# nulltea/hyper-greco

Measured on AMD Instinct MI355X. Metric: GKR prove ms, n=32768 k=16 Goldilocks; achieved HBM GB/s vs roofline, lower is better.
Workload: dtype u64; 1 GPU; GKR prove (sk_encryption_circuit.rs:444-457) of the BFV sk-enc circuit, n=32768 k=16 Goldilocks/GoldilocksExt2, a new witness every step (4 seeded synthetic witnesses in rotation), node tables resident in HBM; witnesses=4, n=32768, k=16, field=goldilocks, parallelism=dp1: one independent proof per GPU, no data-path collective, proof_bytes=149488

## Files before the change

hyper-greco_amd/csrc/kernels.hip:

```cpp
#include <hip/hip_runtime.h>
#include <cstring>
#include <algorithm>
#include <stdexcept>
#include <string>
#include <type_traits>
#include "kernels.hpp"
#include "gl_wide.hpp"
#include "derive_math.hpp"

namespace hg {
namespace dev {

constexpr int TPB = 256;

template <int CTRL, int ROW_MASK>
__device__ __forceinline__ u64 dpp_u64(u64 v) {
    u32 lo = (u32)__builtin_amdgcn_update_dpp(0, (int)(u32)v, CTRL, ROW_MASK, 0xF, false);
    u32 hi = (u32)__builtin_amdgcn_update_dpp(0, (int)(u32)(v >> 32), CTRL, ROW_MASK, 0xF, false);
    return ((u64)hi << 32) | lo;
}
__device__ __forceinline__ u64 wave_sum_u64(u64 v) {
    v = gl_add(v, dpp_u64<0x111, 0xF>(v));
    v = gl_add(v, dpp_u64<0x112, 0xF>(v));
    v = gl_add(v, dpp_u64<0x114, 0xF>(v));
    v = gl_add(v, dpp_u64<0x118, 0xF>(v));
    v = gl_add(v, dpp_u64<0x142, 0xA>(v));
    v = gl_add(v, dpp_u64<0x143, 0xC>(v));
    u32 lo = (u32)__builtin_amdgcn_readlane((int)(u32)v, 63), hi = (u32)__builtin_amdgcn_readlane((int)(u32)(v >> 32), 63);
    return ((u64)hi << 32) | lo;
}
__device__ __forceinline__ E2 wave_sum(E2 v) { return e2(wave_sum_u64(v.c0), wave_sum_u64(v.c1)); }
__device__ __forceinline__ E2 block_sum(E2 v, E2* sm) {
    v = wave_sum(v);
    int lane = threadIdx.x & 63, wave = threadIdx.x >> 6;
    __syncthreads();
    if (lane == 0) sm[wave] = v;
    __syncthreads();
    if (threadIdx.x == 0) {
        for (int w = 1; w < TPB / 64; w++) v = e2_add(v, sm[w]);
    }
    return v;
}

static size_t st_min_threads() { return 65536; }
#ifndef HG_TEST_ST_MAX_BLOCKS
#define HG_TEST_ST_MAX_BLOCKS 512
#endif
static int st_max_blocks() { return HG_TEST_ST_MAX_BLOCKS; }

static inline int grid_for(size_t work_items) {
    size_t b = (work_items + TPB - 1) / TPB;
    if (b < 1) b = 1;
    return (int)(b > (size_t)SC_MAX_BLOCKS ? SC_MAX_BLOCKS : b);
}

template <typename T> struct Val;
template <> struct Val<u64> {
    static __device__ __forceinline__ u64 add(u64 a, u64 b) { return gl_add(a, b); }
    static __device__ __forceinline__ u64 sub(u64 a, u64 b) { return gl_sub(a, b); }
    static __device__ __forceinline__ u64 mul(u64 a, u64 b) { return gl_mul(a, b); }
    static __device__ __forceinline__ E2 scale(E2 c, u64 a) { return e2_mul_f(c, a); }
    static __device__ __forceinline__ E2 fold(u64 x, u64 d, E2 r) { return e2_add_f(e2_mul_f(r, d), x); }
    static __device__ __forceinline__ E2 lift(u64 a) { return e2(a, 0); }
    static __device__ __forceinline__ u64 zero() { return 0; }
};
template <> struct Val<E2> {
    static __device__ __forceinline__ E2 add(E2 a, E2 b) { return e2_add(a, b); }
    static __device__ __forceinline__ E2 sub(E2 a, E2 b) { return e2_sub(a, b); }
    static __device__ __forceinline__ E2 mul(E2 a, E2 b) { return e2_mul(a, b); }
    static __device__ __forceinline__ E2 scale(E2 c, E2 a) { return e2_mul(c, a); }
    static __device__ __forceinline__ E2 fold(E2 x, E2 d, E2 r) { return e2_add(x, e2_mul(r, d)); }
    static __device__ __forceinline__ E2 lift(E2 a) { return a; }
    static __device__ __forceinline__ E2 zero() { return e2_zero(); }
};

typedef unsigned long long u64x2_t __attribute__((ext_vector_type(2)));
#define HG_GLOBAL(T, p) (reinterpret_cast<__attribute__((address_space(1))) T*>((unsigned long long)(p)))
template <bool GIO = true>
__device__ __forceinline__ u64x2_t load16(const void* p) {
    if constexpr (GIO) return *HG_GLOBAL(const u64x2_t, p);
    else return *reinterpret_cast<const u64x2_t*>(p);
}
template <bool GIO = true>
__device__ __forceinline__ void store16(void* p, u64 a, u64 b) {
    u64x2_t w; w.x = a; w.y = b;
    if constexpr (GIO) *HG_GLOBAL(u64x2_t, p) = w;
    else *reinterpret_cast<u64x2_t*>(p) = w;
}
template <typename T, bool GIO = true>
__device__ __forceinline__ void load_pair(const T* p, T& x, T& y) {
    if constexpr (std::is_same<T, u64>::value) {
        const u64x2_t v = load16<GIO>(p);
        x = v.x; y = v.y;
    } else {
        const u64x2_t a = load16<GIO>(p), b = load16<GIO>(p + 1);
        x = e2(a.x, a.y); y = e2(b.x, b.y);
    }
}
template <typename T, bool NATURAL, bool GIO = true>
__device__ __forceinline__ void load_xy(const T* tab, size_t j, size_t half, T& x, T& y) {
    if constexpr (NATURAL || std::is_same<T, u64>::value) load_pair<T, GIO>(tab + 2 * j, x, y);
    else {
        const u64x2_t a = load16<GIO>(tab + j), b = load16<GIO>(tab + half + j);
        x = e2(a.x, a.y); y = e2(b.x, b.y);
    }
}
__device__ __forceinline__ size_t dpos(size_t j, size_t len) { return (j & 1) * (len >> 1) + (j >> 1); }
template <bool GIO = true>
__device__ __forceinline__ void store_e2(E2* p, E2 v) { store16<GIO>(p, v.c0, v.c1); }
template <bool GIO = true>
__device__ __forceinline__ void store_e2_nt(E2* p, E2 v) {
    u64x2_t w; w.x = v.c0; w.y = v.c1;
    if constexpr (GIO) __builtin_nontemporal_store(w, HG_GLOBAL(u64x2_t, p));
    else *reinterpret_cast<u64x2_t*>(p) = w;
}
__device__ __forceinline__ void store_u64x2(u64* p, u64 a, u64 b) { store16<true>(p, a, b); }
__device__ __forceinline__ E2 gload_e2(const E2* p) {
    const u64x2_t v = *HG_GLOBAL(const u64x2_t, p);
    return e2(v.x, v.y);
}
__device__ __forceinline__ u64 gload_u64(const u64* p) { return *HG_GLOBAL(const u64, p); }
__device__ __forceinline__ void gstore_e2(E2* p, E2 v) { store_e2(p, v); }

struct GpFirstAcc { WAcc a0, b0, a1, b1, ai, bi; };
__device__ __forceinline__ GpFirstAcc gp_first_acc_zero() {
    GpFirstAcc A;
    A.a0 = wacc_zero(); A.b0 = wacc_zero(); A.a1 = wacc_zero(); A.b1 = wacc_zero(); A.ai = wacc_zero(); A.bi = wacc_zero();
    return A;
}
template <bool WANT_Q, bool GIO = true>
__device__ __forceinline__ void gp_first_pair(GpFirstAcc& A, u64 xl, u64 yl, u64 xr, u64 yr, E2 gm, E2 gr, E2 r, bool summed,
                                              E2* __restrict__ out_l, E2* __restrict__ out_r, u64* __restrict__ nxt, u64& q0, u64& q1) {
    const u64 dl = gl_sub(yl, xl), dr = gl_sub(yr, xr);
    if (WANT_Q || summed || nxt) {
        q0 = gl_mul(xl, xr); q1 = gl_mul(yl, yr);
        if (nxt) store_u64x2(nxt, q0, q1);
        if (summed) {
            const u64 qi = gl_mul(dl, dr);
            wmac2(A.a0, gm.c0, q0, A.b0, gm.c1, q0);
            wmac2(A.a1, gm.c0, q1, A.b1, gm.c1, q1);
            wmac2(A.ai, gm.c0, qi, A.bi, gm.c1, qi);
        }
    }
    const WAcc f0 = wacc_pair_init(0, gm.c0, xl, gr.c0, dl), f1 = wacc_pair_init(0, gm.c1, xl, gr.c1, dl);
    store_e2_nt<GIO>(out_l, e2(wreduce(f0), wreduce(f1)));
    const WAcc h0 = wacc_mul_init(xr, r.c0, dr), h1 = wacc_mul_init(0, r.c1, dr);
    store_e2_nt<GIO>(out_r, e2(wreduce(h0), wreduce(h1)));
}
__device__ __forceinline__ void emit_rows(u64* __restrict__ next_level, size_t row_stride, size_t at, u64 mask, ulonglong2 q) {
    while (mask) {
        const int t = __ffsll((long long)mask) - 1;
        mask &= mask - 1;
        store_u64x2(next_level + (size_t)t * row_stride + at, q.x, q.y);
    }
}
__device__ __forceinline__ void gp_first_acc_reduce(const GpFirstAcc& A, E2& s0, E2& s2, E2& s3) {
    s0 = e2(wreduce(A.a0), wreduce(A.b0)); s2 = e2(wreduce(A.a1), wreduce(A.b1)); s3 = e2(wreduce(A.ai), wreduce(A.bi));
}

template <bool SLOT, bool GIO>
__device__ __forceinline__ void gp_first_round_body(const u64* __restrict__ in, size_t in_stride, E2* __restrict__ out, size_t out_stride, int ntab, size_t half, E2 r,
                                                    const E2* __restrict__ pw, const E2* __restrict__ pwr, int jb_log2, E2* __restrict__ red, E2* acc,
                                                    size_t first_tile, size_t tile_step, bool p0_only, u64* __restrict__ next_level, const StJob* __restrict__ mirror) {
    const int BD = blockDim.x, tid = threadIdx.x;
    const int G = BD >> jb_log2;
    const int jj = tid & ((1 << jb_log2) - 1), g = tid >> jb_log2;
    const size_t ntiles = half >> jb_log2;
    const int nb = ntab >> 1;
    const E2* __restrict__ slotw = SLOT ? mirror->slotw : nullptr;
    const u64* __restrict__ emask = !SLOT ? nullptr : next_level ? mirror->emit_mask : reinterpret_cast<const u64*>(mirror->slotw);
    const int slot_ng = SLOT ? mirror->slot_ng : 0, slot_shift = SLOT ? mirror->slot_shift : 0;
    struct Item { u64 xl, yl, xr, yr; E2 gm, gr; u64 em; };
    auto any_item = [] {
        const u64 z = 0, u = __builtin_nondeterministic_value(z);
        return Item{u, u, u, u, e2(u, u), e2(u, u), u};
    };
    auto fetch = [&](size_t tile, int i, Item& it) {
        const size_t j = (tile << jb_log2) + jj;
        load_xy<u64, true, GIO>(in + (size_t)(2 * i) * in_stride, j, half, it.xl, it.yl);
        load_xy<u64, true, GIO>(in + (size_t)(2 * i + 1) * in_stride, j, half, it.xr, it.yr);
        it.em = 0;
        if constexpr (SLOT) {
            const size_t at = (size_t)i * slot_ng + (((tile << jb_log2) * 2) >> slot_shift);
            it.gm = gload_e2(slotw + 2 * at); it.gr = gload_e2(slotw + 2 * at + 1);
            it.em = gload_u64(emask + at);
        } else if constexpr (GIO) { it.gm = gload_e2(pw + i); it.gr = gload_e2(pwr + i); }
        else { it.gm = pw[i]; it.gr = pwr[i]; }
    };
    const bool active = g < nb && first_tile < ntiles;
    Item cur = any_item();
    if (active) fetch(first_tile, g, cur);
    for (size_t tile = first_tile; tile < ntiles; tile += tile_step) {
        const size_t j = (tile << jb_log2) + jj;
        const size_t jo = dpos(j, half);
        GpFirstAcc A = gp_first_acc_zero();
        u64 p0 = 0, p2 = 0, p3 = 0;
        if (active) for (int i = g; i < nb; i += G) {
            const bool more_i = i + G < nb, more_t = tile + tile_step < ntiles;
            Item nxt;
            fetch(more_i || !more_t ? tile : tile + tile_step, more_i ? i + G : g, nxt);
            if (i == 0) { const u64 dl = gl_sub(cur.yl, cur.xl); p0 = cur.xl; p2 = gl_add(cur.yl, dl); p3 = gl_add(p2, dl); }
            u64 q0, q1;
            if constexpr (SLOT) {
                gp_first_pair<true, GIO>(A, cur.xl, cur.yl, cur.xr, cur.yr, cur.gm, cur.gr, r, !(p0_only && i == 0), out + (size_t)(2 * i) * out_stride + jo,
                                         out + (size_t)(2 * i + 1) * out_stride + jo, nullptr, q0, q1);
                if (next_level) emit_rows(next_level, in_stride, 2 * j, cur.em, make_ulonglong2(q0, q1));
            } else {
                gp_first_pair<false, GIO>(A, cur.xl, cur.yl, cur.xr, cur.yr, cur.gm, cur.gr, r, !(p0_only && i == 0), out + (size_t)(2 * i) * out_stride + jo,
                                          out + (size_t)(2 * i + 1) * out_stride + jo, next_level ? next_level + (size_t)i * in_stride + 2 * j : nullptr, q0, q1);
            }
            cur = nxt;
        }
        E2 s0, s2, s3;
        gp_first_acc_reduce(A, s0, s2, s3);
        if (G > 1) {
            red[tid] = s0; red[BD + tid] = s2; red[2 * BD + tid] = s3;
            __syncthreads();
            if (g == 0) {
                const int gmax = G < nb ? G : nb;
                for (int gg = 1; gg < gmax; gg++) {
                    int o = (gg << jb_log2) + jj;
                    s0 = e2_add(s0, red[o]); s2 = e2_add(s2, red[BD + o]); s3 = e2_add(s3, red[2 * BD + o]);
                }
            }
            __syncthreads();
        }
        if (g == 0) {
            const E2 P1x2 = e2_dbl(s2), Pix2 = e2_dbl(s3);
            const E2 q2 = e2_add(e2_sub(P1x2, s0), Pix2);
            const E2 q3 = e2_add(e2_sub(e2_add(P1x2, s2), e2_dbl(s0)), e2_add(e2_dbl(Pix2), Pix2));
            acc[0] = e2_add(acc[0], e2_mul_f(s0, p0));
            acc[1] = e2_add(acc[1], e2_mul_f(q2, p2));
            acc[2] = e2_add(acc[2], e2_mul_f(q3, p3));
        }
    }
}

struct GpItemE2 { E2 xl, yl, xr, yr; };
__device__ __forceinline__ GpItemE2 gp_item_any() {
    const u64 z = 0, u = __builtin_nondeterministic_value(z);
    return GpItemE2{e2(u, u), e2(u, u), e2(u, u), e2(u, u)};
}
template <int KIND, typename T, bool FIRST, bool SLOT = false, bool GIO = true, int MODE = 0>
__device__ __forceinline__ void sc_round_body(const T* __restrict__ in, size_t in_stride, E2* __restrict__ out,
                                              size_t out_stride, int ntab, size_t half, E2 r, const E2* __restrict__ pw, const E2* __restrict__ pwr,
                                              int jb_log2, E2* __restrict__ red, E2* acc, size_t first_tile, size_t tile_step,
                                              bool p0_only = false, u64* __restrict__ next_level = nullptr, const StJob* __restrict__ mirror = nullptr) {
    using V = Val<T>;
    if constexpr (KIND == SC_GRANDPROD && FIRST && std::is_same<T, u64>::value) {
        gp_first_round_body<SLOT, GIO>(in, in_stride, out, out_stride, ntab, half, r, pw, pwr, jb_log2, red, acc, first_tile, tile_step, p0_only, next_level, mirror);
        return;
    }
    static_assert(MODE == 0 || (KIND == SC_GRANDPROD && !FIRST && std::is_same<T, E2>::value), "split rounds: grand product, Ext2 tables");
    const int BD = blockDim.x, tid = threadIdx.x;
    const int G = BD >> jb_log2;
    const int jj = tid & ((1 << jb_log2) - 1), g = tid >> jb_log2;
    const size_t ntiles = half >> jb_log2;
    [[maybe_unused]] GpItemE2 gp_cur = gp_item_any();
    constexpr bool COL_WIDE = KIND != SC_GRANDPROD && (std::is_same<T, u64>::value || !GIO);
    [[maybe_unused]] W2 col0 = w2_zero(), col2 = w2_zero();
    [[maybe_unused]] int col_trips = 0;
    for (size_t tile = first_tile; tile < ntiles; tile += tile_step) {
        const size_t j = (tile << jb_log2) + jj;
        const size_t jo = dpos(j, half);
        if constexpr (KIND == SC_GRANDPROD) {
            E2 s0 = e2_zero(), s2 = e2_zero(), s3 = e2_zero();
            T p0 = V::zero(), p2 = V::zero(), p3 = V::zero();
            const int nb = ntab >> 1;
            if constexpr (!FIRST && std::is_same<T, E2>::value) {
                WE2 w0 = we2_zero(), w1 = we2_zero(), wi = we2_zero();
                const FoldR fr = fold_r(r);
                auto fetch = [&](size_t tl, int i, GpItemE2& it) {
                    const size_t jn = (tl << jb_log2) + jj;
                    load_xy<E2, false, GIO>(in + (size_t)(2 * i) * in_stride, jn, half, it.xl, it.yl);
                    load_xy<E2, false, GIO>(in + (size_t)(2 * i + 1) * in_stride, jn, half, it.xr, it.yr);
                };
                if (g < nb && tile == first_tile) fetch(tile, g, gp_cur);
                if (g < nb) for (int i = g; i < nb; i += G) {
                    const bool more_i = i + G < nb, more_t = tile + tile_step < ntiles;
                    GpItemE2 nxt;
                    fetch(more_i || !more_t ? tile : tile + tile_step, more_i ? i + G : g, nxt);
                    const E2 xl = gp_cur.xl, yl = gp_cur.yl, xr = gp_cur.xr, yr = gp_cur.yr;
                    E2 dl = e2_sub(yl, xl), dr = e2_sub(yr, xr);
                    if (i == 0) { p0 = xl; p2 = e2_add(yl, dl); p3 = e2_add(p2, dl); }
                    if (MODE != 1 && !(p0_only && i == 0)) {
                        we2_mac(w0, xl, xr);
                        we2_mac(w1, yl, yr);
                        we2_mac(wi, dl, dr);
                    }
                    if (MODE != 2) {
                        store_e2<GIO>(out + (size_t)(2 * i) * out_stride + jo, e2_fold_wide(xl, dl, fr));
                        store_e2<GIO>(out + (size_t)(2 * i + 1) * out_stride + jo, e2_fold_wide(xr, dr, fr));
                    }
                    gp_cur = nxt;
                }
                if (MODE != 1) { s0 = we2_reduce(w0); s2 = we2_reduce(w1); s3 = we2_reduce(wi); }
                if (mirror && g == 0) {
                    E2 x, y;
                    load_xy<E2, false, GIO>(in + (size_t)(2 * nb) * in_stride, j, half, x, y);
                    if (MODE != 1) {
                        s0 = e2_add(s0, e2_add(e2_mul(mirror->mk1, x), mirror->mk2));
                        s2 = e2_add(s2, e2_add(e2_mul(mirror->mk1, y), mirror->mk2));
                    }
                    if (MODE != 2) store_e2<GIO>(out + (size_t)(2 * nb) * out_stride + jo, e2_fold_wide(x, e2_sub(y, x), fr));
                }
            } else {
            for (int i = g; i < nb; i += G) {
                T xl, yl, xr, yr;
                load_xy<T, FIRST, GIO>(in + (size_t)(2 * i) * in_stride, j, half, xl, yl);
                load_xy<T, FIRST, GIO>(in + (size_t)(2 * i + 1) * in_stride, j, half, xr, yr);
                T dl = V::sub(yl, xl), dr = V::sub(yr, xr);
                if (i == 0) { p0 = xl; p2 = V::add(yl, dl); p3 = V::add(p2, dl); }
                const bool summed = !(p0_only && i == 0);
                E2 gm = pw[i];
                if (summed) {
                    s0 = e2_add(s0, V::scale(gm, V::mul(xl, xr)));
                    s2 = e2_add(s2, V::scale(gm, V::mul(yl, yr)));
                    s3 = e2_add(s3, V::scale(gm, V::mul(dl, dr)));
                }
                store_e2<GIO>(out + (size_t)(2 * i) * out_stride + jo, e2_add(V::scale(gm, xl), V::scale(pwr[i], dl)));
                store_e2<GIO>(out + (size_t)(2 * i + 1) * out_stride + jo, V::fold(xr, dr, r));
            }
            }
            if constexpr (MODE == 1) continue;
            if (G > 1) {
                red[tid] = s0; red[BD + tid] = s2; red[2 * BD + tid] = s3;
                __syncthreads();
                if (g == 0) {
                    const int gmax = G < nb ? G : nb;
                    for (int gg = 1; gg < gmax; gg++) {
                        int o = (gg << jb_log2) + jj;
                        s0 = e2_add(s0, red[o]); s2 = e2_add(s2, red[BD + o]); s3 = e2_add(s3, red[2 * BD + o]);
                    }
                }
                __syncthreads();
            }
            if (g == 0) {
                E2 P0 = s0, P1 = s2, Pi = s3;
                E2 P1x2 = e2_dbl(P1), Pix2 = e2_dbl(Pi);
                E2 q2 = e2_add(e2_sub(P1x2, P0), Pix2);
                E2 q3 = e2_add(e2_sub(e2_add(P1x2, P1), e2_dbl(P0)), e2_add(e2_dbl(Pix2), Pix2));
                acc[0] = e2_add(acc[0], V::scale(P0, p0));
                acc[1] = e2_add(acc[1], V::scale(q2, p2));
                acc[2] = e2_add(acc[2], V::scale(q3, p3));
            }
        } else {
            T s0 = V::zero(), s2 = V::zero(), p0 = V::zero(), p2 = V::zero();
            if constexpr (FIRST && std::is_same<T, u64>::value) {
                WAcc w0 = wacc_zero(), w2 = wacc_zero();
                for (int i = g; i < ntab; i += G) {
                    u64 x, y;
                    load_xy<u64, true, GIO>(in + (size_t)i * in_stride, j, half, x, y);
                    u64 d = gl_sub(y, x);
                    u64 v2 = gl_add(y, d);
                    if (i == 0) { p0 = x; p2 = v2; }
                    const u64 m = pw[i].c0;
                    const E2 mr = pwr[i];
                    if (!(p0_only && i == 0)) wmac2(w0, m, x, w2, m, v2);
                    const WAcc f0 = wacc_pair_init(0, m, x, mr.c0, d), f1 = wacc_mul_init(0, mr.c1, d);
                    store_e2<GIO>(out + (size_t)i * out_stride + jo, e2(wreduce(f0), wreduce(f1)));
                }
                s0 = wreduce(w0); s2 = wreduce(w2);
            } else if constexpr (!FIRST && std::is_same<T, E2>::value) {
                const FoldR fr = fold_r(r);
                for (int i = g; i < ntab; i += G) {
                    E2 x, y;
                    load_xy<E2, false, GIO>(in + (size_t)i * in_stride, j, half, x, y);
                    E2 d = e2_sub(y, x);
                    E2 v2 = e2_add(y, d);
                    if (i == 0) { p0 = x; p2 = v2; }
                    if (!(p0_only && i == 0)) { s0 = e2_add(s0, x); s2 = e2_add(s2, v2); }
                    store_e2<GIO>(out + (size_t)i * out_stride + jo, e2_fold_wide(x, d, fr));
                }
            } else {
            for (int i = g; i < ntab; i += G) {
                T x, y;
                load_xy<T, FIRST, GIO>(in + (size_t)i * in_stride, j, half, x, y);
                T d = V::sub(y, x);
                T v2 = V::add(y, d);
                if (i == 0) { p0 = x; p2 = v2; }
                const bool summed = !(p0_only && i == 0);
                if constexpr (FIRST) {
                    u64 m = pw[i].c0;
                    if constexpr (std::is_same<T, u64>::value) {
                        if (summed) { s0 = gl_add(s0, gl_mul(m, x)); s2 = gl_add(s2, gl_mul(m, v2)); }
                        store_e2<GIO>(out + (size_t)i * out_stride + jo, e2_add_f(e2_mul_f(pwr[i], d), gl_mul(m, x)));
                    } else {
                        if (summed) { s0 = e2_add(s0, e2_mul_f(x, m)); s2 = e2_add(s2, e2_mul_f(v2, m)); }
                        store_e2<GIO>(out + (size_t)i * out_stride + jo, e2_mul_f(V::fold(x, d, r), m));
                    }
                } else {
                    if (summed) { s0 = V::add(s0, x); s2 = V::add(s2, v2); }
                    store_e2<GIO>(out + (size_t)i * out_stride + jo, V::fold(x, d, r));
                }
            }
            }
            E2 t0 = V::lift(s0), t2 = V::lift(s2);
            if (G > 1) {
                red[tid] = t0; red[BD + tid] = t2;
                __syncthreads();
                if (g == 0) {
                    const int gmax = G < ntab ? G : ntab;
                    for (int gg = 1; gg < gmax; gg++) {
                        int o = (gg << jb_log2) + jj;
                        t0 = e2_add(t0, red[o]); t2 = e2_add(t2, red[BD + o]);
                    }
                }
                __syncthreads();
            }
            if (g == 0) {
                if constexpr (!COL_WIDE) {
                    acc[0] = e2_add(acc[0], e2_mul(V::lift(p0), t0));
                    acc[1] = e2_add(acc[1], e2_mul(V::lift(p2), t2));
                } else {
                    if constexpr (std::is_same<T, u64>::value) { w2_mac_f(col0, t0, p0); w2_mac_f(col2, t2, p2); }
                    else { w2_mac(col0, p0, t0); w2_mac(col2, p2, t2); }
                    if (++col_trips == WFLUSH_TRIPS) { col0 = w2_from(w2_reduce(col0)); col2 = w2_from(w2_reduce(col2)); col_trips = 0; }
                }
            }
        }
    }
    if constexpr (COL_WIDE) {
        if (g == 0) { acc[0] = e2_add(acc[0], w2_reduce(col0)); acc[1] = e2_add(acc[1], w2_reduce(col2)); }
    }
}

__device__ __forceinline__ E2 block_sum_n(E2 v, E2* sm ) {
    v = wave_sum(v);
    const int lane = threadIdx.x & 63, wave = threadIdx.x >> 6, nw = (blockDim.x + 63) >> 6;
    __syncthreads();
    if (lane == 0) sm[wave] = v;
    __syncthreads();
    if (threadIdx.x == 0) for (int w = 1; w < nw; w++) v = e2_add(v, sm[w]);
    return v;
}

constexpr int SM_SLOTS = 96;
extern __shared__ E2 dyn_lds[];
template <int N>
__device__ __forceinline__ void block_sum_multi(E2 (&v)[N], E2* sm ) {
    const int lane = threadIdx.x & 63, wave = threadIdx.x >> 6, nw = (blockDim.x + 63) >> 6;
#pragma unroll
    for (int k = 0; k < N; k++) v[k] = wave_sum(v[k]);
    __syncthreads();
    if (lane == 0) {
#pragma unroll
        for (int k = 0; k < N; k++) sm[wave * N + k] = v[k];
    }
    __syncthreads();
    if (threadIdx.x == 0)
        for (int w = 1; w < nw; w++) {
#pragma unroll
            for (int k = 0; k < N; k++) v[k] = e2_add(v[k], sm[w * N + k]);
        }
}

__device__ __forceinline__ void part_store(E2* p, E2 v) {
    __hip_atomic_store(&p->c0, v.c0, __ATOMIC_RELAXED, __HIP_MEMORY_SCOPE_AGENT);
    __hip_atomic_store(&p->c1, v.c1, __ATOMIC_RELAXED, __HIP_MEMORY_SCOPE_AGENT);
}
__device__ __forceinline__ E2 part_load(const E2* p) {
    return e2(__hip_atomic_load(&p->c0, __ATOMIC_RELAXED, __HIP_MEMORY_SCOPE_AGENT), __hip_atomic_load(&p->c1, __ATOMIC_RELAXED, __HIP_MEMORY_SCOPE_AGENT));
}
__device__ __forceinline__ unsigned* tickets_of(E2* partials) { return reinterpret_cast<unsigned*>(partials + PARTIALS_E2); }
struct NoPost { __device__ __forceinline__ void operator()(E2*) const {} };
template <typename Post = NoPost>
__device__ __forceinline__ void finish_partials(E2* p, int per, unsigned* ticket, E2* __restrict__ out, E2* sm ,
                                                int nblocks = -1, Post post = Post()) {
    __shared__ unsigned s_last;
    if (nblocks < 0) nblocks = (int)gridDim.x;
    if (threadIdx.x == 0) {
#if !defined(HG_STRICT_TICKETS) && defined(__HIP_DEVICE_COMPILE__) && !defined(__gfx950__) && !defined(__gfx942__)
#error "the vmcnt-ordered ticket below is only valid on gfx942 / gfx950 (stores tracked by vmcnt, sc1 stores written through); build other architectures with -DHG_STRICT_TICKETS"
#endif
#ifdef HG_STRICT_TICKETS
        unsigned t = __hip_atomic_fetch_add(ticket, 1u, __ATOMIC_ACQ_REL, __HIP_MEMORY_SCOPE_AGENT);
#else
        asm volatile("s_waitcnt vmcnt(0)" ::: "memory");
        unsigned t = __hip_atomic_fetch_add(ticket, 1u, __ATOMIC_RELAXED, __HIP_MEMORY_SCOPE_AGENT);
#endif
        s_last = (t == (unsigned)nblocks - 1) ? 1u : 0u;
    }
    __syncthreads();
    if (!s_last) return;
    __builtin_amdgcn_fence(__ATOMIC_ACQUIRE, "agent");
    constexpr int PER_MAX = 6;
    for (int v0 = 0; v0 < per; v0 += PER_MAX) {
        E2 a[PER_MAX];
#pragma unroll
        for (int v = 0; v < PER_MAX; v++) a[v] = e2_zero();
        for (int b = threadIdx.x; b < nblocks; b += blockDim.x) {
            E2 t[PER_MAX];
#pragma unroll
            for (int v = 0; v < PER_MAX; v++) if (v0 + v < per) t[v] = part_load(p + (size_t)b * per + v0 + v);
#pragma unroll
            for (int v = 0; v < PER_MAX; v++) if (v0 + v < per) a[v] = e2_add(a[v], t[v]);
        }
#pragma unroll
        for (int v = 0; v < PER_MAX; v++) if (v0 + v < per) a[v] = block_sum_n(a[v], sm);
        if (threadIdx.x == 0) {
            if constexpr (!std::is_same<Post, NoPost>::value) post(a);
#pragma unroll
            for (int v = 0; v < PER_MAX; v++) if (v0 + v < per) out[v0 + v] = a[v];
        }
    }
    if (threadIdx.x == 0) __hip_atomic_store(ticket, 0u, __ATOMIC_RELAXED, __HIP_MEMORY_SCOPE_AGENT);
}

__device__ __forceinline__ void st_io(const StJob& J, int rd, const void*& in, size_t& in_stride, E2*& out) {
    const size_t h = (size_t)1 << (J.nvars - 1 - rd);
    if (rd == 0) { in = J.in; in_stride = J.in_stride; }
    else { in = J.buf[(rd - 1) & 1]; in_stride = 2 * h; }
    out = rd == J.nvars - 1 ? J.final_out : J.buf[rd & 1];
}

__device__ __forceinline__ int find_item(const StItem* __restrict__ items, int nitems, int blk) {
    const int l = threadIdx.x & 63;
    const int b0 = l < nitems ? items[l].blk0 : 0x7fffffff;
    const unsigned long long m = __ballot(b0 <= blk);
    return __builtin_amdgcn_readfirstlane(__popcll(m) - 1);
}
template <int KIND, typename T, bool SLOT = false, int MODE = 0>
__global__ __launch_bounds__(256) void k_st_step(const StJob* __restrict__ jobs, const StItem* __restrict__ items, int nitems,
                                                 const E2* __restrict__ chal, E2* __restrict__ partials, E2* __restrict__ res) {
    constexpr int NV = KIND == SC_GRANDPROD ? 3 : 2;
    const int y = find_item(items, nitems, blockIdx.x);
    const StItem& I = items[y];
    const StJob& J = jobs[I.job];
    const int h_log2 = I.h_log2, jb_log2 = I.jb_log2;
    const int rd = J.nvars - 1 - h_log2;
    const size_t half = (size_t)1 << h_log2;
    const int nblocks = I.nblk, bx = (int)blockIdx.x - I.blk0;
    const void* in = I.in; const size_t in_stride = I.in_stride; E2* out = I.out;
    E2* sm = dyn_lds;
    E2* red = dyn_lds + SM_SLOTS;
    E2 acc[NV];
#pragma unroll
    for (int t = 0; t < NV; t++) acc[t] = e2_zero();
    if (rd == 0) sc_round_body<KIND, T, true, SLOT>(reinterpret_cast<const T*>(in), in_stride, out, half, J.ntab, half, chal[J.r_off + rd], J.pw, J.pwr, jb_log2, red, acc, bx, nblocks, J.p0_only != 0, J.next_level,
                                                    SLOT ? &J : nullptr);
    else sc_round_body<KIND, T, false, false, true, MODE>(reinterpret_cast<const T*>(in), in_stride, out, half, J.ntab, half, chal[J.r_off + rd], J.pw, J.pwr, jb_log2, red, acc, bx, nblocks, J.p0_only != 0, nullptr,
                                                          J.mirror ? &J : nullptr);
    if constexpr (MODE == 1) return;
    E2* part = partials + (size_t)y * SC_MAX_BLOCKS * NV;
    block_sum_multi<NV>(acc, sm);
    if (threadIdx.x == 0) {
#pragma unroll
        for (int t = 0; t < NV; t++) {
            if (nblocks == 1) res[J.sums_slot + (size_t)rd * NV + t] = acc[t];
            else part_store(part + (size_t)bx * NV + t, acc[t]);
        }
    }
    if (nblocks > 1) finish_partials(part, NV, tickets_of(partials) + y * 32, res + J.sums_slot + (size_t)rd * NV, sm, nblocks);
}
__device__ __forceinline__ u64 limb_word(const u64* __restrict__ input, const uint8_t* __restrict__ seg_lookup, int seg_shift, size_t rows,
                                         const u64* lookup_mask, size_t j) {
    return j < rows ? input[j] & lookup_mask[seg_lookup[j >> seg_shift]] : 0;
}
__device__ __forceinline__ u32 limb_of(u64 word, int c) { return (u32)(word >> (16 * c)) & 0xFFFF; }
template <typename S>
__device__ __forceinline__ ulonglong2 limb_pair(const S& H, size_t j2, int c) {
    if (j2 >= H.rows) return make_ulonglong2(0, 0);
    const ulonglong2 w = *reinterpret_cast<const ulonglong2*>(H.input + j2);
    const u64 m = H.lookup_mask[H.seg_lookup[j2 >> H.seg_shift]];
    return make_ulonglong2(limb_of(w.x & m, c), limb_of(w.y & m, c));
}
LimbSrc limb_src(const LassoDev& L, const u64* input) {
    LimbSrc S;
    memset(&S, 0, sizeof(S));
    S.input = input; S.seg_lookup = L.seg_lookup; S.seg_shift = L.seg_shift; S.rows = L.rows;
    memcpy(S.lookup_mask, L.lookup_mask, sizeof(S.lookup_mask));
    return S;
}
template <bool MIRROR, bool RECOMP, bool SLOT = false>
#ifndef HG_HASH_SLOT_WAVES
#define HG_HASH_SLOT_WAVES 3
#endif
__global__ __launch_bounds__(256) __attribute__((amdgpu_waves_per_eu(SLOT ? HG_HASH_SLOT_WAVES : 3, SLOT ? HG_HASH_SLOT_WAVES : 3))) void k_gp_first_hash(const StJob* __restrict__ job, const StItem* __restrict__ item,
                                                       const E2* __restrict__ chal, E2* __restrict__ partials, E2* __restrict__ res) {
    const StJob& J = *job;
    const StItem& I = *item;
    const GpHashSrc& H = *J.hash_src;
    const int h_log2 = I.h_log2;
    const size_t half = (size_t)1 << h_log2;
    const size_t hN = half << 1;
    const size_t ntiles = half >> 8;
    const int nblocks = I.nblk, bx = (int)blockIdx.x;
    E2* __restrict__ out = I.out;
    const E2 r = chal[J.r_off];
    const bool p0_only = J.p0_only != 0;
    [[maybe_unused]] constexpr bool mirror = MIRROR;
    const u64 gamma = H.gamma, gamma2 = H.gamma2, tau = H.tau;
    E2 acc[3] = {e2_zero(), e2_zero(), e2_zero()};
    for (size_t tile = bx; tile < ntiles; tile += nblocks) {
        const size_t j = (tile << 8) + threadIdx.x;
        const size_t jo = dpos(j, half);
        GpFirstAcc A = gp_first_acc_zero();
        E2 Sx = e2_zero(), Sy = e2_zero();
        u64 p0 = 0, p2 = 0, p3 = 0;
        int cur_chunk = -1;
        u64 c0 = 0, c1 = 0, c2 = 0, c3 = 0;
        u32 a01 = 0, a23 = 0;
        u32 uses_lo = 0, uses_hi = 0;
        if constexpr (RECOMP) {
            if (2 * j < H.rows) uses_lo = (u32)H.lookup_uses[H.seg_lookup[(2 * j) >> H.seg_shift]];
            if (hN + 2 * j < H.rows) uses_hi = (u32)H.lookup_uses[H.seg_lookup[(hN + 2 * j) >> H.seg_shift]];
        }
        [[maybe_unused]] const int sp = SLOT ? (int)((tile << 9) >> H.seg_shift) : 0;
        for (int m = 0; m < (SLOT ? H.nslots : H.nmem); m++) {
            [[maybe_unused]] int slot_v = m;
            int mi = m;
            if constexpr (SLOT) {
                mi = H.rep[(size_t)m * H.npairs + sp];
                if (mi == 255) {
                    store_e2_nt(out + (size_t)(2 * m) * half + jo, e2_zero());
                    store_e2_nt(out + (size_t)(2 * m + 1) * half + jo, e2_zero());
                    continue;
                }
            }
            const GpHashMem M = H.mems[mi];
            if (M.chunk != cur_chunk) {
                cur_chunk = M.chunk;
                const u64* __restrict__ ts = H.ts[cur_chunk];
                ulonglong2 dl, dh;
                if (H.limb_sh) { dl = limb_pair(H, 2 * j, cur_chunk); dh = limb_pair(H, hN + 2 * j, cur_chunk); }
                else {
                    const u64* __restrict__ dim = H.dim[cur_chunk];
                    dl = *reinterpret_cast<const ulonglong2*>(dim + 2 * j); dh = *reinterpret_cast<const ulonglong2*>(dim + hN + 2 * j);
                }
                const ulonglong2 tl = *reinterpret_cast<const ulonglong2*>(ts + 2 * j), th = *reinterpret_cast<const ulonglong2*>(ts + hN + 2 * j);
                c0 = gl_sub(gl_add(dl.x, gl_mul_small(gamma2, (u32)tl.x)), tau); c1 = gl_sub(gl_add(dl.y, gl_mul_small(gamma2, (u32)tl.y)), tau);
                c2 = gl_sub(gl_add(dh.x, gl_mul_small(gamma2, (u32)th.x)), tau); c3 = gl_sub(gl_add(dh.y, gl_mul_small(gamma2, (u32)th.y)), tau);
                if constexpr (RECOMP) { a01 = (u32)dl.x | ((u32)dl.y << 16); a23 = (u32)dh.x | ((u32)dh.y << 16); }
            }
            u32 e0, e1, e2v, e3;
            if constexpr (RECOMP) {
                const u32 cut = M.cutoff;
                const bool ul = (uses_lo >> M.mem) & 1, uh = (uses_hi >> M.mem) & 1;
                e0 = a01 & 0xFFFF; e1 = a01 >> 16; e2v = a23 & 0xFFFF; e3 = a23 >> 16;
                e0 = (ul && e0 < cut) ? e0 : 0; e1 = (ul && e1 < cut) ? e1 : 0;
                e2v = (uh && e2v < cut) ? e2v : 0; e3 = (uh && e3 < cut) ? e3 : 0;
            } else {
                const ulonglong2 el = *reinterpret_cast<const ulonglong2*>(M.ep + 2 * j), eh = *reinterpret_cast<const ulonglong2*>(M.ep + hN + 2 * j);
                e0 = (u32)el.x; e1 = (u32)el.y; e2v = (u32)eh.x; e3 = (u32)eh.y;
            }
            u64 xl = gl_add(c0, gl_mul_small(gamma, e0)), yl = gl_add(c1, gl_mul_small(gamma, e1));
            u64 xr = gl_add(c2, gl_mul_small(gamma, e2v)), yr = gl_add(c3, gl_mul_small(gamma, e3));
            if constexpr (SLOT) {
                const int i = M.rd_row;
                if (i == 0) { const u64 d = gl_sub(yl, xl); p0 = xl; p2 = gl_add(yl, d); p3 = gl_add(p2, d); }
                const size_t at = (size_t)slot_v * H.npairs + sp;
                const E2 gm = H.slotw[2 * at], gr = H.slotw[2 * at + 1];
                u64 q0, q1;
                const bool summed = !(p0_only && slot_v == 0);
                gp_first_pair<true>(A, xl, yl, xr, yr, gm, gr, r, summed, out + (size_t)(2 * slot_v) * half + jo, out + (size_t)(2 * slot_v + 1) * half + jo, nullptr, q0, q1);
                if (summed) {
                    const u64 hx = gl_add(xl, xr), hy = gl_add(yl, yr);
                    Sx = e2_add(Sx, e2_mul_f(gm, hx));
                    Sy = e2_add(Sy, e2_mul_f(gm, hy));
                }
                if (J.next_level) {
                    emit_rows(J.next_level, hN, 2 * j, H.emit_rd[at], make_ulonglong2(q0, q1));
                    xl = gl_add(xl, gamma2); yl = gl_add(yl, gamma2); xr = gl_add(xr, gamma2); yr = gl_add(yr, gamma2);
                    emit_rows(J.next_level, hN, 2 * j, H.emit_wr[at], make_ulonglong2(gl_mul(xl, xr), gl_mul(yl, yr)));
                }
            } else {
            if (M.rd_row >= 0) {
                const int i = M.rd_row;
                if (i == 0) { const u64 d = gl_sub(yl, xl); p0 = xl; p2 = gl_add(yl, d); p3 = gl_add(p2, d); }
                u64 q0, q1;
                gp_first_pair<false>(A, xl, yl, xr, yr, J.pw[i], J.pwr[i], r, !(p0_only && i == 0), out + (size_t)(2 * i) * half + jo,
                                     out + (size_t)(2 * i + 1) * half + jo, J.next_level ? J.next_level + (size_t)i * hN + 2 * j : nullptr, q0, q1);
                if constexpr (MIRROR) if (!(p0_only && i == 0)) {
                    const E2 gm = J.pw[i];
                    const u64 hx = gl_add(xl, xr), hy = gl_add(yl, yr);
                    Sx = e2_add(Sx, e2_mul_f(gm, hx));
                    Sy = e2_add(Sy, e2_mul_f(gm, hy));
                }
            }
            if (M.wr_row >= 0) {
                const int i = M.wr_row;
                xl = gl_add(xl, gamma2); yl = gl_add(yl, gamma2); xr = gl_add(xr, gamma2); yr = gl_add(yr, gamma2);
                if constexpr (!MIRROR) {
                    u64 q0, q1;
                    gp_first_pair<false>(A, xl, yl, xr, yr, J.pw[i], J.pwr[i], r, true, out + (size_t)(2 * i) * half + jo,
                                         out + (size_t)(2 * i + 1) * half + jo, J.next_level ? J.next_level + (size_t)i * hN + 2 * j : nullptr, q0, q1);
                } else if (J.next_level)
                    *reinterpret_cast<ulonglong2*>(J.next_level + (size_t)i * hN + 2 * j) = make_ulonglong2(gl_mul(xl, xr), gl_mul(yl, yr));
            }
            }
        }
        E2 s0, s2, s3;
        gp_first_acc_reduce(A, s0, s2, s3);
        if constexpr (MIRROR) {
            s0 = e2_add(s0, e2_add(e2_mul(J.mk1, Sx), J.mk2));
            s2 = e2_add(s2, e2_add(e2_mul(J.mk1, Sy), J.mk2));
            store_e2_nt(out + (size_t)(J.ntab - 1) * half + jo, e2_add(Sx, e2_mul(r, e2_sub(Sy, Sx))));
        }
        const E2 P1x2 = e2_dbl(s2), Pix2 = e2_dbl(s3);
        const E2 q2 = e2_add(e2_sub(P1x2, s0), Pix2);
        const E2 q3 = e2_add(e2_sub(e2_add(P1x2, s2), e2_dbl(s0)), e2_add(e2_dbl(Pix2), Pix2));
        acc[0] = e2_add(acc[0], e2_mul_f(s0, p0));
        acc[1] = e2_add(acc[1], e2_mul_f(q2, p2));
        acc[2] = e2_add(acc[2], e2_mul_f(q3, p3));
    }
    E2* sm = dyn_lds;
    block_sum_multi<3>(acc, sm);
    if (threadIdx.x == 0) {
#pragma unroll
        for (int t = 0; t < 3; t++) {
            if (nblocks == 1) res[J.sums_slot + t] = acc[t];
            else part_store(partials + (size_t)bx * 3 + t, acc[t]);
        }
    }
    if (nblocks > 1) finish_partials(partials, 3, tickets_of(partials), res + J.sums_slot, sm, nblocks);
}
struct HashSlotD {
    E2 gm, gr;
    u64 erd, ewr;
    int chunk, pad0;
    int rd_row, mem;
    u32 cutoff;
    int valid;
    int pad[2];
};
static_assert(sizeof(HashSlotD) == 80, "HashSlotD layout");
__global__ __launch_bounds__(256) __attribute__((amdgpu_waves_per_eu(2, 2))) void k_gp_first_hash_slot(const StJob* __restrict__ job, const StItem* __restrict__ item, const E2* __restrict__ chal,
                                                           E2* __restrict__ partials, E2* __restrict__ res) {
    const StJob& J = *job;
    const StItem& I = *item;
    const GpHashSrc& H = *J.hash_src;
    const size_t half = (size_t)1 << I.h_log2;
    const size_t hN = half << 1;
    const size_t ntiles = half >> 8;
    const int nblocks = I.nblk, bx = (int)blockIdx.x, tid = threadIdx.x;
    E2* __restrict__ out = I.out;
    const E2 r = chal[J.r_off];
    const bool p0_only = J.p0_only != 0;
    const u64 gamma = H.gamma, gamma2 = H.gamma2, tau = H.tau;
    const int nslots = H.nslots, npairs = H.npairs, seg_shift = H.seg_shift;
    u64* __restrict__ next_level = J.next_level;
    const int ntab = J.ntab;
    const E2 mk1 = J.mk1, mk2 = J.mk2;
    const size_t per = (ntiles + nblocks - 1) / nblocks;
    const size_t t_lo = (size_t)bx * per, t_hi = t_lo + per < ntiles ? t_lo + per : ntiles;
    __shared__ HashSlotD D[64];
    __shared__ const u64* s_dim[4];
    __shared__ const u64* s_ts[4];
    __shared__ int s_ng, s_glo[65], s_gchunk[64], s_gsh[64];
    __shared__ u32 s_uses[2];
    __shared__ u64 s_mask[2];
    int staged_sp = -1;
    auto stage = [&](int sp, size_t tile) {
        __syncthreads();
        if (tid < nslots) {
            HashSlotD d;
            const size_t at = (size_t)tid * npairs + sp;
            const int mi = H.rep[at];
            d.gm = gload_e2(H.slotw + 2 * at); d.gr = gload_e2(H.slotw + 2 * at + 1);
            d.erd = next_level ? gload_u64(H.emit_rd + at) : 0; d.ewr = next_level ? gload_u64(H.emit_wr + at) : 0;
            d.valid = mi != 255;
            d.chunk = -1; d.pad0 = 0; d.rd_row = 0; d.mem = 0; d.cutoff = 0; d.pad[0] = d.pad[1] = 0;
            if (d.valid) { const GpHashMem M = H.mems[mi]; d.chunk = M.chunk; d.rd_row = M.rd_row; d.mem = M.mem; d.cutoff = M.cutoff; }
            D[tid] = d;
        }
        if (tid < 4) { s_dim[tid] = H.dim[tid]; s_ts[tid] = H.ts[tid]; }
        if (tid == 64) {
            const size_t p = tile << 9;
            const int l0 = p < H.rows ? H.seg_lookup[p >> seg_shift] : -1, l1 = hN + p < H.rows ? H.seg_lookup[(hN + p) >> seg_shift] : -1;
            s_uses[0] = l0 >= 0 ? (u32)H.lookup_uses[l0] : 0u;
            s_uses[1] = l1 >= 0 ? (u32)H.lookup_uses[l1] : 0u;
            s_mask[0] = l0 >= 0 ? H.lookup_mask[l0] : 0;
            s_mask[1] = l1 >= 0 ? H.lookup_mask[l1] : 0;
        }
        __syncthreads();
        if (tid == 0) {
            int ng = 0, cur = -1;
            for (int m = 0; m < nslots; m++) {
                if (!D[m].valid || D[m].chunk == cur) continue;
                cur = D[m].chunk;
                s_glo[ng] = ng == 0 ? 0 : m; s_gchunk[ng] = cur; s_gsh[ng] = H.limb_sh * cur; ng++;
            }
            if (ng == 0) { s_glo[0] = 0; s_gchunk[0] = 0; s_gsh[0] = 0; ng = 1; }
            s_glo[ng] = nslots;
            s_ng = ng;
        }
        __syncthreads();
        staged_sp = sp;
    };
    struct Raw { u64x2_t dl, dh, tl, th; };
    auto request = [&](size_t tile, int chunk, Raw& w) {
        const size_t j = (tile << 8) + tid;
        const u64* __restrict__ dim = s_dim[chunk];
        const u64* __restrict__ ts = s_ts[chunk];
        w.dl = load16<true>(dim + 2 * j); w.dh = load16<true>(dim + hN + 2 * j);
        w.tl = load16<true>(ts + 2 * j); w.th = load16<true>(ts + hN + 2 * j);
    };
    E2 acc[3] = {e2_zero(), e2_zero(), e2_zero()};
    Raw nxt;
    if (t_lo < t_hi) {
        stage((int)((t_lo << 9) >> seg_shift), t_lo);
        request(t_lo, s_gchunk[0], nxt);
    }
    for (size_t tile = t_lo; tile < t_hi; tile++) {
        const int sp = (int)((tile << 9) >> seg_shift);
        if (sp != staged_sp) {
            stage(sp, tile);
            request(tile, s_gchunk[0], nxt);
        }
        const size_t j = (tile << 8) + tid;
        const size_t jo = dpos(j, half);
        const u32 uses_lo = 2 * j < H.rows ? s_uses[0] : 0u, uses_hi = hN + 2 * j < H.rows ? s_uses[1] : 0u;
        GpFirstAcc A = gp_first_acc_zero();
        E2 Sx = e2_zero(), Sy = e2_zero();
        u64 p0 = 0, p2 = 0, p3 = 0;
        const int ng = s_ng;
        for (int k = 0; k < ng; k++) {
        const int shc = __builtin_amdgcn_readfirstlane(s_gsh[k]);
        const bool up = (shc & 32) != 0;
        const int sh16 = shc & 16;
        const u32 ml = (u32)__builtin_amdgcn_readfirstlane((int)(s_mask[0] >> (up ? 32 : 0))) >> sh16 & 0xFFFF;
        const u32 mh = (u32)__builtin_amdgcn_readfirstlane((int)(s_mask[1] >> (up ? 32 : 0))) >> sh16 & 0xFFFF;
        const u32 d0 = ((up ? (u32)(nxt.dl.x >> 32) : (u32)nxt.dl.x) >> sh16) & ml, d1 = ((up ? (u32)(nxt.dl.y >> 32) : (u32)nxt.dl.y) >> sh16) & ml;
        const u32 d2 = ((up ? (u32)(nxt.dh.x >> 32) : (u32)nxt.dh.x) >> sh16) & mh, d3 = ((up ? (u32)(nxt.dh.y >> 32) : (u32)nxt.dh.y) >> sh16) & mh;
        const u64 c0 = gl_sub(gl_add((u64)d0, gl_mul_small(gamma2, (u32)nxt.tl.x)), tau), c1 = gl_sub(gl_add((u64)d1, gl_mul_small(gamma2, (u32)nxt.tl.y)), tau);
        const u64 c2 = gl_sub(gl_add((u64)d2, gl_mul_small(gamma2, (u32)nxt.th.x)), tau), c3 = gl_sub(gl_add((u64)d3, gl_mul_small(gamma2, (u32)nxt.th.y)), tau);
        const u32 a01 = d0 | (d1 << 16), a23 = d2 | (d3 << 16);
        {
            const bool more_k = k + 1 < ng, more_t = tile + 1 < t_hi;
            request(more_k || !more_t ? tile : tile + 1, s_gchunk[more_k ? k + 1 : (more_t ? 0 : k)], nxt);
        }
        const int m_hi = s_glo[k + 1];
        for (int m = s_glo[k]; m < m_hi; m++) {
            const int valid = __builtin_amdgcn_readfirstlane(D[m].valid);
            if (!valid) {
                store_e2_nt(out + (size_t)(2 * m) * half + jo, e2_zero());
                store_e2_nt(out + (size_t)(2 * m + 1) * half + jo, e2_zero());
                continue;
            }
            const u32 cut = (u32)__builtin_amdgcn_readfirstlane((int)D[m].cutoff);
            const int mem = __builtin_amdgcn_readfirstlane(D[m].mem), rd_row = __builtin_amdgcn_readfirstlane(D[m].rd_row);
            const bool ul = (uses_lo >> mem) & 1, uh = (uses_hi >> mem) & 1;
            u32 e0 = a01 & 0xFFFF, e1 = a01 >> 16, e2v = a23 & 0xFFFF, e3 = a23 >> 16;
            e0 = (ul && e0 < cut) ? e0 : 0; e1 = (ul && e1 < cut) ? e1 : 0;
            e2v = (uh && e2v < cut) ? e2v : 0; e3 = (uh && e3 < cut) ? e3 : 0;
            u64 xl = gl_add(c0, gl_mul_small(gamma, e0)), yl = gl_add(c1, gl_mul_small(gamma, e1));
            u64 xr = gl_add(c2, gl_mul_small(gamma, e2v)), yr = gl_add(c3, gl_mul_small(gamma, e3));
            if (rd_row == 0) { const u64 d = gl_sub(yl, xl); p0 = xl; p2 = gl_add(yl, d); p3 = gl_add(p2, d); }
            const E2 gm = D[m].gm, gr = D[m].gr;
            u64 q0, q1;
            const bool summed = !(p0_only && m == 0);
            gp_first_pair<true>(A, xl, yl, xr, yr, gm, gr, r, summed, out + (size_t)(2 * m) * half + jo, out + (size_t)(2 * m + 1) * half + jo, nullptr, q0, q1);
            if (summed) {
                const u64 hx = gl_add(xl, xr), hy = gl_add(yl, yr);
                Sx = e2_add(Sx, e2_mul_f(gm, hx));
                Sy = e2_add(Sy, e2_mul_f(gm, hy));
            }
            if (next_level) {
                const u64 erd = ((u64)(u32)__builtin_amdgcn_readfirstlane((int)(D[m].erd >> 32)) << 32) | (u32)__builtin_amdgcn_readfirstlane((int)D[m].erd);
                const u64 ewr = ((u64)(u32)__builtin_amdgcn_readfirstlane((int)(D[m].ewr >> 32)) << 32) | (u32)__builtin_amdgcn_readfirstlane((int)D[m].ewr);
                emit_rows(next_level, hN, 2 * j, erd, make_ulonglong2(q0, q1));
                xl = gl_add(xl, gamma2); yl = gl_add(yl, gamma2); xr = gl_add(xr, gamma2); yr = gl_add(yr, gamma2);
                emit_rows(next_level, hN, 2 * j, ewr, make_ulonglong2(gl_mul(xl, xr), gl_mul(yl, yr)));
            }
        }
        }
        E2 s0, s2, s3;
        gp_first_acc_reduce(A, s0, s2, s3);
        s0 = e2_add(s0, e2_add(e2_mul(mk1, Sx), mk2));
        s2 = e2_add(s2, e2_add(e2_mul(mk1, Sy), mk2));
        store_e2_nt(out + (size_t)(ntab - 1) * half + jo, e2_add(Sx, e2_mul(r, e2_sub(Sy, Sx))));
        const E2 P1x2 = e2_dbl(s2), Pix2 = e2_dbl(s3);
        const E2 q2 = e2_add(e2_sub(P1x2, s0), Pix2);
        const E2 q3 = e2_add(e2_sub(e2_add(P1x2, s2), e2_dbl(s0)), e2_add(e2_dbl(Pix2), Pix2));
        acc[0] = e2_add(acc[0], e2_mul_f(s0, p0));
        acc[1] = e2_add(acc[1], e2_mul_f(q2, p2));
        acc[2] = e2_add(acc[2], e2_mul_f(q3, p3));
    }
    E2* sm = dyn_lds;
    block_sum_multi<3>(acc, sm);
    if (threadIdx.x == 0) {
#pragma unroll
        for (int t = 0; t < 3; t++) {
            if (nblocks == 1) res[J.sums_slot + t] = acc[t];
            else part_store(partials + (size_t)bx * 3 + t, acc[t]);
        }
    }
    if (nblocks > 1) finish_partials(partials, 3, tickets_of(partials), res + J.sums_slot, sm, nblocks);
}
static inline size_t sc_lds_bytes(int nv, int bd);
void st_first_hash(hipStream_t st, const StJob* job, const StItem* item, int grid, bool mirror, bool recomp, const E2* chal, E2* partials, E2* res, bool slot) {
    const size_t lds = sc_lds_bytes(0, 256);
    if (slot) {
        if (!mirror) throw std::runtime_error("st_first_hash: the slot form is a mirrored job");
        if (recomp) k_gp_first_hash_slot<<<grid, 256, lds, st>>>(job, item, chal, partials, res);
        else k_gp_first_hash<true, false, true><<<grid, 256, lds, st>>>(job, item, chal, partials, res);
    } else if (recomp) {
        if (mirror) k_gp_first_hash<true, true><<<grid, 256, lds, st>>>(job, item, chal, partials, res);
        else k_gp_first_hash<false, true><<<grid, 256, lds, st>>>(job, item, chal, partials, res);
    } else {
        if (mirror) k_gp_first_hash<true, false><<<grid, 256, lds, st>>>(job, item, chal, partials, res);
        else k_gp_first_hash<false, false><<<grid, 256, lds, st>>>(job, item, chal, partials, res);
    }
}

__device__ __forceinline__ u64 swap_lane_u64(u64 v) {
    u32 lo = (u32)v, hi = (u32)(v >> 32);
    lo = (u32)__builtin_amdgcn_mov_dpp((int)lo, 0xB1, 0xF, 0xF, true);
    hi = (u32)__builtin_amdgcn_mov_dpp((int)hi, 0xB1, 0xF, 0xF, true);
    return ((u64)hi << 32) | lo;
}
__device__ __forceinline__ E2 swap_lane(E2 v) { return e2(swap_lane_u64(v.c0), swap_lane_u64(v.c1)); }
__device__ __forceinline__ E2 gp_combine(E2 P0, E2 P1, E2 Pi, E2 p0, E2 p2, E2 p3, E2& a0, E2& a1, E2& a2) {
    E2 P1x2 = e2_dbl(P1), Pix2 = e2_dbl(Pi);
    E2 q2 = e2_add(e2_sub(P1x2, P0), Pix2);
    E2 q3 = e2_add(e2_sub(e2_add(P1x2, P1), e2_dbl(P0)), e2_add(e2_dbl(Pix2), Pix2));
    a0 = e2_add(a0, e2_mul(P0, p0));
    a1 = e2_add(a1, e2_mul(q2, p2));
    a2 = e2_add(a2, e2_mul(q3, p3));
    return q2;
}
__global__ __launch_bounds__(256) void k_st_step2(const StJob* __restrict__ jobs, const StItem* __restrict__ items, int nitems,
                                                  const E2* __restrict__ chal, E2* __restrict__ partials, E2* __restrict__ res) {
    const int y = find_item(items, nitems, blockIdx.x);
    const StItem& I = items[y];
    const StJob& J = jobs[I.job];
    const int h_log2 = I.h_log2;
    const int rd = J.nvars - 1 - h_log2;
    const size_t half = (size_t)1 << h_log2, half2 = half >> 1;
    const size_t ntiles = half >> 8;
    const int nblocks = I.nblk, bx = (int)blockIdx.x - I.blk0;
    const E2* __restrict__ in = reinterpret_cast<const E2*>(I.in);
    const size_t in_stride = I.in_stride;
    E2* __restrict__ out = I.out;
    const int nb = J.ntab >> 1;
    const bool p0_only = J.p0_only != 0;
    const int tid = threadIdx.x;
    const bool odd = tid & 1;
    const FoldR fa = fold_r(chal[J.r_off + rd]);
    const E2 rb = chal[J.r_off + rd + 1];
    const FoldR fb = fold_r(odd ? e2_sub(e2_one(), rb) : rb);
    E2 acc[6];
#pragma unroll
    for (int t = 0; t < 6; t++) acc[t] = e2_zero();
    GpItemE2 cur = gp_item_any();
    if ((size_t)bx < ntiles) {
        load_xy<E2, false>(in, ((size_t)bx << 8) + tid, half, cur.xl, cur.yl);
        load_xy<E2, false>(in + in_stride, ((size_t)bx << 8) + tid, half, cur.xr, cur.yr);
    }
    for (size_t tile = bx; tile < ntiles; tile += nblocks) {
        const size_t j = (tile << 8) + tid;
        const size_t j2 = j >> 1;
        const size_t jo2 = dpos(j2, half2);
        WE2 w0 = we2_zero(), w1 = we2_zero(), wi = we2_zero();
        W2 vm = w2_zero();
        WAcc vi = wacc_zero();
        E2 p0 = e2_zero(), p2 = e2_zero(), p3 = e2_zero(), q0 = e2_zero(), q2 = e2_zero(), q3 = e2_zero();
        if (J.mirror) {
            E2 x, y;
            load_xy<E2, false>(in + (size_t)(2 * nb) * in_stride, j, half, x, y);
            const E2 ms = e2_fold_wide(x, e2_sub(y, x), fa);
            const E2 es = e2_sub(swap_lane(ms), ms);
            const E2 c0 = e2_add(e2_mul(J.mk1, x), J.mk2), c1 = e2_add(e2_mul(J.mk1, y), J.mk2), cm = e2_add(e2_mul(J.mk1, ms), J.mk2);
            w0.A.L = c0.c0; w0.C.L = c0.c1;
            w1.A.L = c1.c0; w1.C.L = c1.c1;
            vm.c0.L = cm.c0; vm.c1.L = cm.c1;
            const E2 fs = e2_fold_wide(ms, es, fb);
            if (!odd) store_e2(out + (size_t)(2 * nb) * half2 + jo2, fs);
        }
        for (int i = 0; i < nb; i++) {
            const bool more_i = i + 1 < nb, more_t = tile + nblocks < ntiles;
            GpItemE2 nxt;
            {
                const size_t jn = ((more_i || !more_t ? tile : tile + nblocks) << 8) + tid;
                const int in_ = more_i ? i + 1 : 0;
                load_xy<E2, false>(in + (size_t)(2 * in_) * in_stride, jn, half, nxt.xl, nxt.yl);
                load_xy<E2, false>(in + (size_t)(2 * in_ + 1) * in_stride, jn, half, nxt.xr, nxt.yr);
            }
            const E2 xl = cur.xl, yl = cur.yl, xr = cur.xr, yr = cur.yr;
            const E2 dl = e2_sub(yl, xl), dr = e2_sub(yr, xr);
            const bool summed = !(p0_only && i == 0);
            if (i == 0) { p0 = xl; p2 = e2_add(yl, dl); p3 = e2_add(p2, dl); }
            if (summed) { we2_mac(w0, xl, xr); we2_mac(w1, yl, yr); we2_mac(wi, dl, dr); }
            const E2 ml = e2_fold_wide(xl, dl, fa), mr = e2_fold_wide(xr, dr, fa);
            const E2 ol = swap_lane(ml), orr = swap_lane(mr);
            const E2 el = e2_sub(ol, ml), er = e2_sub(orr, mr);
            if (i == 0) {
                const E2 x = odd ? ol : ml, y = odd ? ml : ol;
                const E2 d = e2_sub(y, x);
                q0 = x; q2 = e2_add(y, d); q3 = e2_add(q2, d);
            }
            if (summed) {
                w2_mac(vm, ml, mr);
                const u64 b = odd ? er.c1 : er.c0, d = odd ? er.c0 : er.c1;
                const u64 c = odd ? el.c1 : gl_mul7_lazy(el.c1);
                wmac_pair(vi, el.c0, b, c, d);
            }
            const E2 fx = odd ? mr : ml, fd = odd ? er : el;
            store_e2(out + (size_t)(2 * i + (odd ? 1 : 0)) * half2 + jo2, e2_fold_wide(fx, fd, fb));
            cur = nxt;
        }
        gp_combine(we2_reduce(w0), we2_reduce(w1), we2_reduce(wi), p0, p2, p3, acc[0], acc[1], acc[2]);
        const E2 mine = w2_reduce(vm), other = swap_lane(mine);
        const u64 ip = wreduce(vi), iq = swap_lane_u64(ip);
        if (!odd) gp_combine(mine, other, e2(ip, iq), q0, q2, q3, acc[3], acc[4], acc[5]);
    }
    E2* sm = dyn_lds;
    E2* part = partials + (size_t)y * SC_MAX_BLOCKS * 6;
    block_sum_multi<6>(acc, sm);
    if (threadIdx.x == 0) {
#pragma unroll
        for (int t = 0; t < 6; t++) {
            if (nblocks == 1) res[J.sums_slot + (size_t)rd * 3 + t] = acc[t];
            else part_store(part + (size_t)bx * 6 + t, acc[t]);
        }
    }
    if (nblocks > 1) finish_partials(part, 6, tickets_of(partials) + y * 32, res + J.sums_slot + (size_t)rd * 3, sm, nblocks);
}
__global__ __launch_bounds__(256) void k_col_step2(const StJob* __restrict__ jobs, const StItem* __restrict__ items, int nitems,
                                                   const E2* __restrict__ chal, E2* __restrict__ partials, E2* __restrict__ res) {
    const int y = find_item(items, nitems, blockIdx.x);
    const StItem& I = items[y];
    const StJob& J = jobs[I.job];
    const int h_log2 = I.h_log2;
    const int rd = J.nvars - 1 - h_log2;
    const size_t half = (size_t)1 << h_log2, half2 = half >> 1;
    const size_t ntiles = half >> 8;
    const int nblocks = I.nblk, bx = (int)blockIdx.x - I.blk0;
    const E2* __restrict__ in = reinterpret_cast<const E2*>(I.in);
    const size_t in_stride = I.in_stride;
    E2* __restrict__ out = I.out;
    const int ntab = J.ntab;
    const bool p0_only = J.p0_only != 0;
    const int tid = threadIdx.x;
    const bool odd = tid & 1;
    const FoldR fa = fold_r(chal[J.r_off + rd]);
    const E2 rb = chal[J.r_off + rd + 1];
    const FoldR fb = fold_r(odd ? e2_sub(e2_one(), rb) : rb);
    W2 w0 = w2_zero(), w2 = w2_zero(), wq = w2_zero();
    int trips = 0;
    for (size_t tile = bx; tile < ntiles; tile += nblocks) {
        const size_t j = (tile << 8) + tid;
        const size_t jo2 = dpos(j >> 1, half2);
        E2 s0 = e2_zero(), s2 = e2_zero(), own = e2_zero();
        E2 p0 = e2_zero(), p2 = e2_zero(), q0 = e2_zero(), q2 = e2_zero();
        for (int i = 0; i < ntab; i += 2) {
            const bool two = i + 1 < ntab;
            E2 xa, ya, xb = e2_zero(), yb = e2_zero();
            load_xy<E2, false>(in + (size_t)i * in_stride, j, half, xa, ya);
            if (two) load_xy<E2, false>(in + (size_t)(i + 1) * in_stride, j, half, xb, yb);
            const E2 da = e2_sub(ya, xa), db = e2_sub(yb, xb);
            const E2 va = e2_add(ya, da), vb = e2_add(yb, db);
            if (i == 0) { p0 = xa; p2 = va; }
            if (p0_only && i == 0) { s0 = e2_add(s0, xb); s2 = e2_add(s2, vb); }
            else { s0 = e2_add(s0, e2_add(xa, xb)); s2 = e2_add(s2, e2_add(va, vb)); }
            const E2 ma = e2_fold_wide(xa, da, fa), mb = two ? e2_fold_wide(xb, db, fa) : e2_zero();
            const E2 oa = swap_lane(ma), ob = swap_lane(mb);
            if (i == 0) {
                const E2 x = odd ? oa : ma, yv = odd ? ma : oa;
                q0 = x; q2 = e2_add(yv, e2_sub(yv, x));
            }
            own = e2_add(own, (p0_only && i == 0) ? mb : e2_add(ma, mb));
            const E2 fx = odd ? mb : ma, fd = odd ? e2_sub(ob, mb) : e2_sub(oa, ma);
            if (!odd || two) store_e2(out + (size_t)(i + (odd ? 1 : 0)) * half2 + jo2, e2_fold_wide(fx, fd, fb));
        }
        w2_mac(w0, p0, s0);
        w2_mac(w2, p2, s2);
        const E2 other = swap_lane(own);
        w2_mac(wq, odd ? q2 : q0, odd ? e2_sub(e2_dbl(own), other) : own);
        if (++trips == WFLUSH_TRIPS) { w0 = w2_from(w2_reduce(w0)); w2 = w2_from(w2_reduce(w2)); wq = w2_from(w2_reduce(wq)); trips = 0; }
    }
    const E2 rq = w2_reduce(wq);
    E2 acc[4] = {w2_reduce(w0), w2_reduce(w2), odd ? e2_zero() : rq, odd ? rq : e2_zero()};
    E2* sm = dyn_lds;
    E2* part = partials + (size_t)y * SC_MAX_BLOCKS * 4;
    block_sum_multi<4>(acc, sm);
    if (threadIdx.x == 0) {
#pragma unroll
        for (int t = 0; t < 4; t++) {
            if (nblocks == 1) res[J.sums_slot + (size_t)rd * 2 + t] = acc[t];
            else part_store(part + (size_t)bx * 4 + t, acc[t]);
        }
    }
    if (nblocks > 1) finish_partials(part, 4, tickets_of(partials) + y * 32, res + J.sums_slot + (size_t)rd * 2, sm, nblocks);
}

static inline size_t sc_lds_bytes(int nv, int bd) { return (SM_SLOTS + (size_t)nv * bd) * sizeof(E2); }

constexpr size_t ST_TAIL_LDS_BYTES = 120 * 1024;
constexpr int ST_TAIL_THREADS = 256;
int st_tail_h(int ntab, int nvars) {
    int h = 0;
    while (h + 1 <= nvars - 1 && (size_t)ntab * (((size_t)1 << (h + 1)) + ((size_t)1 << h)) * sizeof(E2) <= ST_TAIL_LDS_BYTES) h++;
    return h;
}
__device__ __forceinline__ void gp_claim_epilogue(const GpClaimEp* __restrict__ ep, const E2* __restrict__ fin, E2* __restrict__ res, E2* sm) {
    const int nb = ep->nb, nread = ep->nread;
    const bool has_next = ep->has_next != 0, has_claims = ep->has_claims != 0;
    const E2 mu = ep->mu;
    const u64 c = ep->c;
    E2* __restrict__ ev = res + ep->evals_slot;
    W2 w = w2_zero();
    for (int b = threadIdx.x; b < nb; b += blockDim.x) {
        const int rb = (nread && b >= nread) ? b - nread : b;
        E2 l = fin[2 * rb], r = fin[2 * rb + 1];
        if (rb > 0) l = e2_mul(l, gload_e2(ep->winv + rb));
        if (rb != b) { l = e2_add_f(l, c); r = e2_add_f(r, c); }
        gstore_e2(ev + 2 * b, l);
        gstore_e2(ev + 2 * b + 1, r);
        const E2 cl = e2_add(l, e2_mul(mu, e2_sub(r, l)));
        if (has_claims) gstore_e2(res + ep->claims_slot + b, cl);
        if (has_next) w2_mac(w, cl, gload_e2(ep->gnext + b));
    }
    if (has_next) {
        const E2 s = block_sum_n(w2_reduce(w), sm);
        if (threadIdx.x == 0) gstore_e2(res + ep->next_slot, s);
    }
}
template <int KIND>
__global__ __launch_bounds__(ST_TAIL_THREADS) void k_st_tail(const StJob* __restrict__ jobs, const StItem* __restrict__ items, const E2* __restrict__ chal,
                                                 E2* __restrict__ res) {
    constexpr int NV = KIND == SC_GRANDPROD ? 3 : 2;
    __shared__ StJob Jl;
    __shared__ StItem Il;
    {
        const StItem* gi = items + blockIdx.x;
        const unsigned* src = reinterpret_cast<const unsigned*>(jobs + gi->job);
        unsigned* dst = reinterpret_cast<unsigned*>(&Jl);
        for (unsigned k = threadIdx.x; k < sizeof(StJob) / 4; k += blockDim.x) dst[k] = src[k];
        if (threadIdx.x < sizeof(StItem) / 4) reinterpret_cast<unsigned*>(&Il)[threadIdx.x] = reinterpret_cast<const unsigned*>(gi)[threadIdx.x];
    }
    __syncthreads();
    const StItem& I = Il;
    if (threadIdx.x == 0 && Il.ntab > 0) Jl.ntab = Il.ntab;
    __syncthreads();
    const StJob& J = Jl;
    E2* sm = dyn_lds;
    E2* red = dyn_lds + SM_SLOTS;
    E2* tab[2];
    const int h0 = J.nvars - 1 - I.rd;
    tab[0] = red + NV * ST_TAIL_THREADS;
    tab[1] = tab[0] + ((size_t)J.ntab << h0);
    const bool p0_only = J.p0_only != 0;
    const StJob* mirror = (KIND == SC_GRANDPROD && J.mirror) ? &J : nullptr;
    const void* in = I.in;
    size_t in_stride = I.in_stride;
    __shared__ E2 keep[3 * 32], rch[32];
    if ((int)threadIdx.x < J.nvars - I.rd) rch[threadIdx.x] = chal[J.r_off + I.rd + threadIdx.x];
    __syncthreads();
#pragma unroll 1
    for (int rd = I.rd; rd < J.nvars; rd++) {
        const int h_log2 = J.nvars - 1 - rd;
        const size_t half = (size_t)1 << h_log2;
        const int jb_log2 = h_log2 < 8 ? h_log2 : 8;
        E2* out = tab[(rd - I.rd) & 1];
        E2 acc[NV];
#pragma unroll
        for (int t = 0; t < NV; t++) acc[t] = e2_zero();
        const E2 r = rch[rd - I.rd];
        if (rd == 0 && J.base) sc_round_body<KIND, u64, true, false, false>(reinterpret_cast<const u64*>(in), in_stride, out, half, J.ntab, half, r, J.pw, J.pwr, jb_log2, red, acc, 0, 1, p0_only);
        else if (rd == 0) sc_round_body<KIND, E2, true, false, false>(reinterpret_cast<const E2*>(in), in_stride, out, half, J.ntab, half, r, J.pw, J.pwr, jb_log2, red, acc, 0, 1, p0_only);
        else sc_round_body<KIND, E2, false, false, false>(reinterpret_cast<const E2*>(in), in_stride, out, half, J.ntab, half, r, J.pw, J.pwr, jb_log2, red, acc, 0, 1, p0_only, nullptr, mirror);
        block_sum_multi<NV>(acc, sm);
        if (threadIdx.x == 0) {
#pragma unroll
            for (int t = 0; t < NV; t++) keep[(rd - I.rd) * NV + t] = acc[t];
        }
        __syncthreads();
        in = out; in_stride = half;
    }
    if ((int)threadIdx.x < (J.nvars - I.rd) * NV) res[J.sums_slot + (size_t)I.rd * NV + threadIdx.x] = keep[threadIdx.x];
    const E2* fin = reinterpret_cast<const E2*>(in);
    if (KIND == SC_GRANDPROD && J.ep) gp_claim_epilogue(J.ep, fin, res, sm);
    else for (int t = threadIdx.x; t < J.ntab; t += blockDim.x) J.final_out[t] = fin[t];
}
__global__ void k_gp_slot_regroup(const E2* __restrict__ in, E2* __restrict__ out, const uint8_t* __restrict__ slot_of, const E2* __restrict__ ratio,
                                  int nrows, int nslots, int npairs, int len_log2, int sh, int has_s) {
    const size_t len = (size_t)1 << len_log2;
    const size_t idx = (size_t)blockIdx.x * blockDim.x + threadIdx.x;
    if (idx >= ((size_t)nrows + has_s) << len_log2) return;
    const int b = (int)(idx >> len_log2);
    const size_t p = idx & (len - 1);
    if (b == nrows) { out[((size_t)(2 * nrows) << len_log2) + p] = in[((size_t)(2 * nslots) << len_log2) + p]; return; }
    const size_t t = p < len / 2 ? 2 * p : 2 * (p - len / 2) + 1;
    const int sp = (int)(t >> sh);
    const int v = slot_of[(size_t)b * npairs + sp];
    const E2 l = in[((size_t)(2 * v) << len_log2) + p], r = in[((size_t)(2 * v + 1) << len_log2) + p];
    out[((size_t)(2 * b) << len_log2) + p] = b == 0 ? l : e2_mul(ratio[(size_t)b * npairs + sp], l);
    out[((size_t)(2 * b + 1) << len_log2) + p] = r;
}
__global__ void k_gp_slot_regroup_jobs(const SlotRegroupJob* __restrict__ jobs) {
    const SlotRegroupJob& J = jobs[blockIdx.y];
    const size_t len = (size_t)1 << J.len_log2;
    const size_t idx = (size_t)blockIdx.x * blockDim.x + threadIdx.x;
    if (idx >= ((size_t)J.nrows + J.has_s) << J.len_log2) return;
    const int b = (int)(idx >> J.len_log2);
    const size_t p = idx & (len - 1);
    if (b == J.nrows) { J.out[((size_t)(2 * J.nrows) << J.len_log2) + p] = J.in[((size_t)(2 * J.nslots) << J.len_log2) + p]; return; }
    const size_t t = p < len / 2 ? 2 * p : 2 * (p - len / 2) + 1;
    const int sp = (int)(t >> J.sh);
    const int v = J.slot_of[(size_t)b * J.npairs + sp];
    const E2 l = J.in[((size_t)(2 * v) << J.len_log2) + p], r = J.in[((size_t)(2 * v + 1) << J.len_log2) + p];
    J.out[((size_t)(2 * b) << J.len_log2) + p] = b == 0 ? l : e2_mul(J.ratio[(size_t)b * J.npairs + sp], l);
    J.out[((size_t)(2 * b + 1) << J.len_log2) + p] = r;
}
void gp_slot_regroup_jobs(hipStream_t st, const SlotRegroupJob* jobs, int njobs, size_t max_entries) {
    if (njobs) k_gp_slot_regroup_jobs<<<dim3((unsigned)((max_entries + 255) / 256), (unsigned)njobs), 256, 0, st>>>(jobs);
}
SlotRegroupJob gp_slot_regroup_job(const E2* in, E2* out, const uint8_t* slot_of, const E2* ratio, int nrows, int nslots, int npairs, int len_log2, bool has_s) {
    int np_log2 = 0;
    while ((1 << np_log2) < npairs) np_log2++;
    SlotRegroupJob J;
    J.in = in; J.out = out; J.slot_of = slot_of; J.ratio = ratio; J.nrows = nrows; J.nslots = nslots; J.npairs = npairs; J.len_log2 = len_log2; J.sh = len_log2 - np_log2; J.has_s = has_s ? 1 : 0;
    return J;
}
void gp_slot_regroup(hipStream_t st, const E2* in, E2* out, const uint8_t* slot_of, const E2* ratio, int nrows, int nslots, int npairs, int len_log2, bool has_s) {
    int np_log2 = 0;
    while ((1 << np_log2) < npairs) np_log2++;
    const size_t n = ((size_t)nrows + (has_s ? 1 : 0)) << len_log2;
    k_gp_slot_regroup<<<(unsigned)((n + 255) / 256), 256, 0, st>>>(in, out, slot_of, ratio, nrows, nslots, npairs, len_log2, len_log2 - np_log2, has_s ? 1 : 0);
}
void st_tail(hipStream_t st, int kind, const StJob* jobs, const StItem* items, int nitems, size_t table_bytes, const E2* chal, E2* res) {
    const size_t lds = (SM_SLOTS + 3 * ST_TAIL_THREADS) * sizeof(E2) + table_bytes;
    static const hipError_t a1 = hipFuncSetAttribute((const void*)k_st_tail<SC_GRANDPROD>, hipFuncAttributeMaxDynamicSharedMemorySize, (int)((SM_SLOTS + 3 * ST_TAIL_THREADS) * sizeof(E2) + ST_TAIL_LDS_BYTES));
    static const hipError_t a2 = hipFuncSetAttribute((const void*)k_st_tail<SC_COLLATION>, hipFuncAttributeMaxDynamicSharedMemorySize, (int)((SM_SLOTS + 3 * ST_TAIL_THREADS) * sizeof(E2) + ST_TAIL_LDS_BYTES));
    (void)a1; (void)a2;
    if (kind == SC_GRANDPROD) k_st_tail<SC_GRANDPROD><<<nitems, ST_TAIL_THREADS, lds, st>>>(jobs, items, chal, res);
    else k_st_tail<SC_COLLATION><<<nitems, ST_TAIL_THREADS, lds, st>>>(jobs, items, chal, res);
}

int st_plan_blocks(StItem* items, int nitems, bool rounds2) {
    size_t total = 0;
    for (int q = 0; q < nitems; q++) total += (size_t)1 << items[q].h_log2;
    int blk = 0;
    for (int q = 0; q < nitems; q++) {
        StItem& I = items[q];
        int jb = 8;
        if (!rounds2) while (jb > 2 && (total << (8 - jb)) < st_min_threads()) jb--;
        if (jb > I.h_log2) jb = I.h_log2;
        const size_t ntiles = ((size_t)1 << I.h_log2) >> jb;
        I.jb_log2 = jb;
        I.blk0 = blk;
        I.nblk = (int)std::min<size_t>(ntiles, (size_t)st_max_blocks());
        blk += I.nblk;
    }
    return blk;
}
void st_step(hipStream_t st, int kind, bool base, const StJob* jobs, const StItem* items, int nitems, int grid, const E2* chal,
             E2* partials, E2* res, bool slot, int mode) {
    const int nv = kind == SC_GRANDPROD ? 3 : 2;
    const size_t lds = sc_lds_bytes(nv, 256);
    if (mode) {
        if (kind != SC_GRANDPROD || base || slot) throw std::runtime_error("st_step: split rounds are grand-product rounds on Ext2 tables");
        if (mode == 1) k_st_step<SC_GRANDPROD, E2, false, 1><<<grid, 256, lds, st>>>(jobs, items, nitems, chal, partials, res);
        else k_st_step<SC_GRANDPROD, E2, false, 2><<<grid, 256, lds, st>>>(jobs, items, nitems, chal, partials, res);
        return;
    }
    if (slot) {
        if (kind != SC_GRANDPROD || !base || nitems != 1) throw std::runtime_error("st_step: a slot-form first round is launched alone");
        k_st_step<SC_GRANDPROD, u64, true><<<grid, 256, lds, st>>>(jobs, items, nitems, chal, partials, res);
    } else if (kind == SC_GRANDPROD) {
        if (base) k_st_step<SC_GRANDPROD, u64><<<grid, 256, lds, st>>>(jobs, items, nitems, chal, partials, res);
        else k_st_step<SC_GRANDPROD, E2><<<grid, 256, lds, st>>>(jobs, items, nitems, chal, partials, res);
    } else {
        if (base) k_st_step<SC_COLLATION, u64><<<grid, 256, lds, st>>>(jobs, items, nitems, chal, partials, res);
        else k_st_step<SC_COLLATION, E2><<<grid, 256, lds, st>>>(jobs, items, nitems, chal, partials, res);
    }
}
void st_step2(hipStream_t st, int kind, const StJob* jobs, const StItem* items, int nitems, int grid, const E2* chal, E2* partials, E2* res) {
    if (kind == SC_GRANDPROD) k_st_step2<<<grid, 256, sc_lds_bytes(0, 256), st>>>(jobs, items, nitems, chal, partials, res);
    else k_col_step2<<<grid, 256, sc_lds_bytes(0, 256), st>>>(jobs, items, nitems, chal, partials, res);
}
__device__ __forceinline__ void ps_io(const PsJob& J, int rd, int rounds, int in_buf, int out_buf, int i, const void*& a, const E2*& b, E2*& oa, E2*& ob) {
    const size_t N = (size_t)1 << J.nvars;
    if (in_buf < 0) { a = J.a[i]; b = J.b[i]; }
    else { size_t len = N >> rd; a = J.bufa[in_buf] + (size_t)i * len; b = J.bufb[in_buf] + (size_t)i * len; }
    if (out_buf < 0) { oa = J.fin_a[i]; ob = J.fin_b[i]; }
    else { size_t len = N >> (rd + rounds); oa = J.bufa[out_buf] + (size_t)i * len; ob = J.bufb[out_buf] + (size_t)i * len; }
}

template <typename TA>
__device__ __forceinline__ void ps_round_body(const PsJob& J, int rd, int in_buf, int out_buf, size_t half, E2 r, int jb_log2, E2& a0, E2& a2,
                                              size_t first_tile, size_t tile_step) {
    using V = Val<TA>;
    const int BD = blockDim.x, tid = threadIdx.x;
    const int G = BD >> jb_log2;
    const int jj = tid & ((1 << jb_log2) - 1), g = tid >> jb_log2;
    const size_t ntiles = half >> jb_log2;
    WE2 w0 = we2_zero(), w2 = we2_zero();
    const FoldR fr = fold_r(r);
    bool touched = false;
    for (size_t tile = first_tile; tile < ntiles; tile += tile_step) {
        const size_t j = (tile << jb_log2) + jj;
        const size_t jo = dpos(j, half);
        for (int i = g; i < J.npairs; i += G) {
            touched = true;
            const void* pa; const E2* pb; E2* oa; E2* ob;
            ps_io(J, rd, 1, in_buf, out_buf, i, pa, pb, oa, ob);
            TA xa, ya;
            E2 xb, yb;
            if (in_buf < 0) {
                load_pair<TA>(reinterpret_cast<const TA*>(pa) + 2 * j, xa, ya);
                load_pair<E2>(pb + 2 * j, xb, yb);
            } else {
                load_xy<TA, false>(reinterpret_cast<const TA*>(pa), j, half, xa, ya);
                load_xy<E2, false>(pb, j, half, xb, yb);
            }
            TA da = V::sub(ya, xa);
            E2 db = e2_sub(yb, xb);
            E2 vb = e2_add(yb, db);
            TA va = V::add(ya, da);
            if constexpr (std::is_same<TA, u64>::value) {
                wmac2(w0.A, xb.c0, xa, w0.C, xb.c1, xa);
                wmac2(w2.A, vb.c0, va, w2.C, vb.c1, va);
                const WAcc f0 = wacc_mul_init(xa, fr.r0, da), f1 = wacc_mul_init(0, fr.r1, da);
                store_e2(oa + jo, e2(wreduce(f0), wreduce(f1)));
            } else {
                we2_mac(w0, xb, xa);
                we2_mac(w2, vb, va);
                store_e2(oa + jo, e2_fold_wide(xa, da, fr));
            }
            store_e2(ob + jo, e2_fold_wide(xb, db, fr));
        }
    }
    if (touched) {
        a0 = e2_add(a0, we2_reduce(w0));
        a2 = e2_add(a2, we2_reduce(w2));
    }
}

__device__ __forceinline__ int find_ps_item(const PsItem* __restrict__ items, int nitems, int blk) {
    const int l = threadIdx.x & 63;
    const int b0 = l < nitems ? items[l].blk0 : 0x7fffffff;
    const unsigned long long m = __ballot(b0 <= blk);
    return __builtin_amdgcn_readfirstlane(__popcll(m) - 1);
}
__global__ __launch_bounds__(256) void k_ps_one(const PsJob* __restrict__ jobs, const PsItem* __restrict__ items, int nitems,
                                                const E2* __restrict__ chal, E2* __restrict__ partials, E2* __restrict__ res) {
    const int y = find_ps_item(items, nitems, blockIdx.x);
    const PsItem& I = items[y];
    const PsJob& J = jobs[I.job];
    const int rd = I.rd;
    const int nblocks = I.nblk, bx = (int)blockIdx.x - I.blk0;
    E2* sm = dyn_lds;
    const size_t half = (size_t)1 << (J.nvars - 1 - rd);
    E2 r = chal[J.r_off + rd];
    E2 a0 = e2_zero(), a2 = e2_zero();
    if (I.in_buf < 0) ps_round_body<u64>(J, rd, I.in_buf, I.out_buf, half, r, I.jb_log2, a0, a2, bx, nblocks);
    else ps_round_body<E2>(J, rd, I.in_buf, I.out_buf, half, r, I.jb_log2, a0, a2, bx, nblocks);
    E2 sv[2] = {a0, a2};
    block_sum_multi<2>(sv, sm);
    const E2 s0 = sv[0], s2 = sv[1];
    E2* part = partials + (size_t)y * SC_MAX_BLOCKS * 4;
    if (threadIdx.x == 0) {
        if (nblocks == 1) { res[J.sums_slot + 2 * rd] = s0; res[J.sums_slot + 2 * rd + 1] = s2; }
        else { part_store(part + (size_t)bx * 2, s0); part_store(part + (size_t)bx * 2 + 1, s2); }
    }
    if (nblocks > 1) finish_partials(part, 2, tickets_of(partials) + y * 32, res + J.sums_slot + 2 * rd, sm, nblocks);
}
template <typename TA>
__device__ __forceinline__ void ps_step2_body(const PsJob& J, const PsItem& I, size_t half, E2 ra, E2 rb, E2* acc , E2* sm) {
    using V = Val<TA>;
    const int tid = threadIdx.x;
    const bool odd = tid & 1;
    const size_t half2 = half >> 1, ntiles = half >> 8;
    const int nblocks = I.nblk, bx = (int)blockIdx.x - I.blk0;
    const FoldR fa = fold_r(ra);
    const FoldR fb = fold_r(odd ? e2_sub(e2_one(), rb) : rb);
    WE2 w0 = we2_zero(), w2 = we2_zero();
    W2 vm = w2_zero();
    WAcc vi = wacc_zero();
    struct Item { TA xa, ya; E2 xb, yb; };
    const int np = J.npairs;
    auto fetch = [&](size_t tl, int i, Item& it) {
        const size_t jn = (tl << 8) + tid;
        const void* pa; const E2* pb; E2* oa; E2* ob;
        ps_io(J, I.rd, 2, I.in_buf, I.out_buf, i, pa, pb, oa, ob);
        if (I.in_buf < 0) {
            load_pair<TA>(reinterpret_cast<const TA*>(pa) + 2 * jn, it.xa, it.ya);
            load_pair<E2>(pb + 2 * jn, it.xb, it.yb);
        } else {
            load_xy<TA, false>(reinterpret_cast<const TA*>(pa), jn, half, it.xa, it.ya);
            load_xy<E2, false>(pb, jn, half, it.xb, it.yb);
        }
    };
    Item cur;
    if ((size_t)bx < ntiles) fetch(bx, 0, cur);
    for (size_t tile = bx; tile < ntiles; tile += nblocks) {
        const size_t j = (tile << 8) + tid;
        const size_t jo2 = dpos(j >> 1, half2);
        for (int i = 0; i < np; i++) {
            const bool more_i = i + 1 < np, more_t = tile + nblocks < ntiles;
            Item nxt;
            fetch(more_i || !more_t ? tile : tile + nblocks, more_i ? i + 1 : 0, nxt);
            const void* pa; const E2* pb; E2* oa; E2* ob;
            ps_io(J, I.rd, 2, I.in_buf, I.out_buf, i, pa, pb, oa, ob);
            const TA xa = cur.xa, ya = cur.ya;
            const E2 xb = cur.xb, yb = cur.yb;
            TA da = V::sub(ya, xa);
            E2 db = e2_sub(yb, xb);
            E2 vb = e2_add(yb, db);
            TA va = V::add(ya, da);
            E2 ma;
            if constexpr (std::is_same<TA, u64>::value) {
                wmac2(w0.A, xb.c0, xa, w0.C, xb.c1, xa);
                wmac2(w2.A, vb.c0, va, w2.C, vb.c1, va);
                const WAcc f0 = wacc_mul_init(xa, fa.r0, da), f1 = wacc_mul_init(0, fa.r1, da);
                ma = e2(wreduce(f0), wreduce(f1));
            } else {
                we2_mac(w0, xb, xa);
                we2_mac(w2, vb, va);
                ma = e2_fold_wide(xa, da, fa);
            }
            const E2 mb = e2_fold_wide(xb, db, fa);
            const E2 oa_ = swap_lane(ma), ob_ = swap_lane(mb);
            const E2 ea = e2_sub(oa_, ma), eb = e2_sub(ob_, mb);
            w2_mac(vm, ma, mb);
            const u64 b = odd ? eb.c1 : eb.c0, d = odd ? eb.c0 : eb.c1;
            const u64 c = odd ? ea.c1 : gl_mul7_lazy(ea.c1);
            wmac_pair(vi, ea.c0, b, c, d);
            const E2 fx = odd ? mb : ma, fd = odd ? eb : ea;
            store_e2((odd ? ob : oa) + jo2, e2_fold_wide(fx, fd, fb));
            cur = nxt;
        }
    }
    acc[0] = we2_reduce(w0);
    acc[1] = we2_reduce(w2);
    const E2 mine = w2_reduce(vm);
    const u64 ip = wreduce(vi);
    E2 v[5] = {acc[0], acc[1], odd ? e2_zero() : mine, odd ? mine : e2_zero(), odd ? e2(0, ip) : e2(ip, 0)};
    block_sum_multi<5>(v, sm);
    acc[0] = v[0]; acc[1] = v[1];
    acc[2] = v[2];
    acc[3] = e2_add(e2_sub(e2_dbl(v[3]), v[2]), e2_dbl(v[4]));
}
__device__ __forceinline__ void w2_mac_pre(W2& w, u64 a0, u64 a1, u64 a17, E2 b) {
    wmac_pair(w.c0, a0, b.c0, a17, b.c1);
    wmac_pair(w.c1, a0, b.c1, a1, b.c0);
}
struct Fold4 { E2 c[4]; u64 c17[4]; };
__device__ __forceinline__ Fold4 fold4(const E2* __restrict__ c) {
    Fold4 f;
#pragma unroll
    for (int p = 0; p < 4; p++) { f.c[p] = c[p]; f.c17[p] = gl_mul7_lazy(f.c[p].c1); }
    return f;
}
__device__ __forceinline__ E2 fold4_apply(const Fold4& f, const u64 (&v)[4]) {
    WAcc a = wacc_mul_init(0, f.c[0].c0, v[0]), b = wacc_mul_init(0, f.c[0].c1, v[0]);
#pragma unroll
    for (int p = 1; p < 4; p++) wmac2(a, f.c[p].c0, v[p], b, f.c[p].c1, v[p]);
    return e2(wreduce(a), wreduce(b));
}
__device__ __forceinline__ E2 fold4_apply(const Fold4& f, const E2 (&v)[4]) {
    WAcc a = wacc_pair_init(0, f.c[0].c0, v[0].c0, f.c17[0], v[0].c1), b = wacc_pair_init(0, f.c[0].c0, v[0].c1, f.c[0].c1, v[0].c0);
#pragma unroll
    for (int p = 1; p < 4; p++) {
        wmac_pair(a, f.c[p].c0, v[p].c0, f.c17[p], v[p].c1);
        wmac_pair(b, f.c[p].c0, v[p].c1, f.c[p].c1, v[p].c0);
    }
    return e2(wreduce(a), wreduce(b));
}
template <typename T>
__device__ __forceinline__ void load4(const T* tab, bool natural, size_t jq, size_t q, T (&v)[4]) {
    if (natural) { load_pair<T>(tab + 4 * jq, v[0], v[1]); load_pair<T>(tab + 4 * jq + 2, v[2], v[3]); }
    else {
#pragma unroll
        for (int p = 0; p < 4; p++) {
            if constexpr (std::is_same<T, u64>::value) v[p] = gload_u64(tab + (size_t)p * q + jq);
            else v[p] = gload_e2(tab + (size_t)p * q + jq);
        }
    }
}
constexpr int PS_EQ_OUT_TAIL = 1;
template <typename TA>
__device__ __forceinline__ bool ps_eq_step2_body(const PsJob& J, const PsItem& I, size_t half, E2* acc , E2* sm) {
    constexpr bool BASE = std::is_same<TA, u64>::value;
    const int tid = threadIdx.x;
    const size_t q = half >> 1, ntiles = q >> 8;
    const int ngroups = I.jb_log2, nblocks = I.nblk / ngroups;
    const int grp = ((int)blockIdx.x - I.blk0) / nblocks, bx = ((int)blockIdx.x - I.blk0) % nblocks;
    const int rd = I.rd, nm = J.eq_n;
    const int gs = (nm + ngroups - 1) / ngroups, m0 = grp * gs, m1 = m0 + gs < nm ? m0 + gs : nm;
    const bool single = J.eq_single != 0, natural = I.in_buf < 0, out_tail = (I.pad & PS_EQ_OUT_TAIL) != 0;
    const bool sums = grp == 0;
    const Fold4 f4 = fold4(J.eq_scal + 2 * J.nvars + 1 + nm + J.nvars + 4 * (rd >> 1));
    const E2* __restrict__ hi = J.eq_suf + (((size_t)1 << (J.nvars - (rd + 10))) - 1);
    const E2* __restrict__ Ain = single ? nullptr : (natural ? J.eqA0 : J.bufA[I.in_buf]);
    const E2 l8 = gload_e2(J.eq_lo + (size_t)(rd + 1) * 384 + tid);
    W2 U[4];
#pragma unroll
    for (int p = 0; p < 4; p++) U[p] = w2_zero();
    auto member_tab = [&](int i) { return natural ? reinterpret_cast<const TA*>(J.a[i]) : reinterpret_cast<const TA*>(J.bufa[I.in_buf]) + (size_t)i * 4 * q; };
    TA cv[4];
    E2 nhv = e2_zero();
    if ((size_t)bx < ntiles && m0 < m1) { load4<TA>(member_tab(m0), natural, ((size_t)bx << 8) + tid, q, cv); nhv = gload_e2(hi + bx); }
    for (size_t tile = bx; tile < ntiles; tile += nblocks) {
        const size_t jq = (tile << 8) + tid;
        const size_t jo = out_tail ? dpos(jq, q) : (jq & 3) * (q >> 2) + (jq >> 2);
        const E2 hv = nhv;
        const bool more = tile + nblocks < ntiles;
        if (more) nhv = gload_e2(hi + tile + nblocks);
        const bool live = (hv.c0 | hv.c1) != 0;
        const u64 h17 = gl_mul7_lazy(hv.c1);
        E2 Av[4];
        if (!single && sums) load4<E2>(Ain, false, jq, q, Av);
        for (int i = m0; i < m1; i++) {
            TA nv[4];
            {
                const bool more_i = i + 1 < m1;
                load4<TA>(member_tab(more_i ? i + 1 : m0), natural, more_i || !more ? jq : ((tile + nblocks) << 8) + tid, q, nv);
            }
            const TA (&v)[4] = cv;
            if (single && live) {
#pragma unroll
                for (int p = 0; p < 4; p++) {
                    if constexpr (BASE) wmac2(U[p].c0, hv.c0, v[p], U[p].c1, hv.c1, v[p]);
                    else w2_mac_pre(U[p], hv.c0, hv.c1, h17, v[p]);
                }
            }
            gstore_e2(J.bufa[I.out_buf] + (size_t)i * q + jo, fold4_apply(f4, v));
#pragma unroll
            for (int p = 0; p < 4; p++) cv[p] = nv[p];
        }
        if (!single && sums) {
            if (live) {
#pragma unroll
                for (int p = 0; p < 4; p++) w2_mac_pre(U[p], hv.c0, hv.c1, h17, Av[p]);
            }
            gstore_e2(J.bufA[I.out_buf] + jo, fold4_apply(f4, Av));
        }
    }
    if (!sums) return false;
    E2 v[4];
#pragma unroll
    for (int p = 0; p < 4; p++) v[p] = e2_mul(l8, w2_reduce(U[p]));
    block_sum_multi<4>(v, sm);
#pragma unroll
    for (int p = 0; p < 4; p++) acc[p] = v[p];
    return true;
}
struct PsEqPost {
    const PsJob* J; int rd; E2 ra;
    __device__ __forceinline__ void operator()(E2* v) const {
        const E2* __restrict__ pre = J->eq_scal + 2 * rd;
        const E2 z = J->eq_scal[2 * J->nvars + 1 + J->eq_n + rd + 1];
        const E2 S0 = e2_add(v[0], e2_mul(z, e2_sub(v[2], v[0]))), S1 = e2_add(v[1], e2_mul(z, e2_sub(v[3], v[1])));
        const E2 T0 = e2_add(v[0], e2_mul(ra, e2_sub(v[1], v[0]))), T1 = e2_add(v[2], e2_mul(ra, e2_sub(v[3], v[2])));
        v[0] = e2_mul(pre[0], S0);
        v[1] = e2_mul(pre[1], e2_sub(e2_dbl(S1), S0));
        v[2] = e2_mul(pre[2], T0);
        v[3] = e2_mul(pre[3], e2_sub(e2_dbl(T1), T0));
    }
};
__global__ __launch_bounds__(256) void k_ps_eq_A(const PsJob* __restrict__ jobs, const int* __restrict__ ids) {
    const PsJob& J = jobs[ids[blockIdx.y]];
    const size_t q = ((size_t)1 << J.nvars) >> 2;
    const E2* __restrict__ kap = J.eq_scal + 2 * J.nvars + 1;
    for (size_t jq = (size_t)blockIdx.x * blockDim.x + threadIdx.x; jq < q; jq += (size_t)gridDim.x * blockDim.x) {
        WAcc w[4][2];
#pragma unroll
        for (int p = 0; p < 4; p++) { w[p][0] = wacc_zero(); w[p][1] = wacc_zero(); }
        u64 nv[4];
        load4<u64>(reinterpret_cast<const u64*>(J.a[0]), true, jq, q, nv);
        for (int i = 0; i < J.eq_n; i++) {
            u64 v[4];
#pragma unroll
            for (int p = 0; p < 4; p++) v[p] = nv[p];
            if (i + 1 < J.eq_n) load4<u64>(reinterpret_cast<const u64*>(J.a[i + 1]), true, jq, q, nv);
            const E2 k = kap[i];
#pragma unroll
            for (int p = 0; p < 4; p++) wmac2(w[p][0], k.c0, v[p], w[p][1], k.c1, v[p]);
        }
#pragma unroll
        for (int p = 0; p < 4; p++) gstore_e2(J.eqA0 + (size_t)p * q + jq, e2(wreduce(w[p][0]), wreduce(w[p][1])));
// ... 1804 lines not shown
```

hyper-greco_amd/csrc/kernels.hpp:

```cpp
#pragma once
#include <hip/hip_runtime.h>
#include <algorithm>
#include "gl_field.hpp"

namespace hg {
namespace dev {

constexpr int SC_MAX_BLOCKS = 1024;
constexpr size_t PARTIALS_E2 = (size_t)SC_MAX_BLOCKS * 6 * 64;
constexpr int PARTIALS_TICKETS = 64 * 32;
constexpr size_t PARTIALS_BYTES = PARTIALS_E2 * sizeof(E2) + PARTIALS_TICKETS * sizeof(unsigned);
constexpr int PS_MAX_PAIRS = 32;
constexpr int PW_MAX = 128;
constexpr int PW_ENTRY_MAX = 64;

struct Powers { E2 v[PW_MAX]; };
constexpr int MAX_CLAIMS = 32;
struct ClaimSet {
    int n;
    int unit_alpha;
    size_t alpha_off;
    size_t point_off[MAX_CLAIMS];
};

enum ScKind { SC_COLLATION = 0, SC_GRANDPROD = 1 };

struct GpHashMem {
    const u64* ep;
    int chunk;
    int rd_row, wr_row;
    u32 cutoff;
    int mem;
};
struct GpHashSrc {
    const u64* dim[4];
    const u64* ts[4];
    const GpHashMem* mems;
    int nmem;
    u64 gamma, gamma2, tau;
    int seg_shift;
    size_t rows;
    const uint8_t* seg_lookup;
    u64 lookup_uses[32];
    const u64* input;
    int limb_sh;
    u64 lookup_mask[32];
    const uint8_t* slot_of;
    const uint8_t* rep;
    const E2* slotw;
    int npairs, nslots;
    const u64* emit_rd;
    const u64* emit_wr;
};
void gp_slot_regroup(hipStream_t st, const E2* in, E2* out, const uint8_t* slot_of, const E2* ratio, int nrows, int nslots, int npairs, int len_log2, bool has_s = true);
struct SlotRegroupJob { const E2* in; E2* out; const uint8_t* slot_of; const E2* ratio; int nrows, nslots, npairs, len_log2, sh, has_s; };
SlotRegroupJob gp_slot_regroup_job(const E2* in, E2* out, const uint8_t* slot_of, const E2* ratio, int nrows, int nslots, int npairs, int len_log2, bool has_s);
void gp_slot_regroup_jobs(hipStream_t st, const SlotRegroupJob* jobs, int njobs, size_t max_entries);
struct GpClaimEp {
    E2 mu;
    u64 c;
    int nb;
    int nread;
    int has_next, has_claims;
    size_t evals_slot, next_slot, claims_slot;
    const E2* winv;
    const E2* gnext;
};
struct StJob {
    const void* in;
    size_t in_stride;
    E2* buf[2];
    E2* final_out;
    const GpClaimEp* ep;
    int kind, ntab, nvars, base;
    int p0_only;
    const E2* slotw;
    const u64* emit_mask;
    int slot_ng, slot_shift;
    int mirror;
    E2 mk1, mk2;
    size_t r_off;
    size_t sums_slot;
    const GpHashSrc* hash_src;
    u64* next_level;
    E2 pw[PW_MAX];
    E2 pwr[PW_MAX];
};
struct StItem {
    int job;
    int h_log2;
    int jb_log2;
    int blk0, nblk;
    const void* in;
    size_t in_stride;
    E2* out;
    int rd, nrounds;
    int ntab;
};
int st_plan_blocks(StItem* items, int nitems, bool rounds2);
void st_step(hipStream_t st, int kind, bool base, const StJob* jobs, const StItem* items, int nitems, int grid, const E2* chal,
             E2* partials, E2* res, bool slot = false, int mode = 0);
void st_first_hash(hipStream_t st, const StJob* job, const StItem* item, int grid, bool mirror, bool recomp, const E2* chal, E2* partials, E2* res, bool slot = false);
void st_step2(hipStream_t st, int kind, const StJob* jobs, const StItem* items, int nitems, int grid, const E2* chal, E2* partials, E2* res);
int st_tail_h(int ntab, int nvars);
void st_tail(hipStream_t st, int kind, const StJob* jobs, const StItem* items, int nitems, size_t table_bytes, const E2* chal, E2* res);
constexpr int ST_STEP2_MIN_H = 9;

struct PsJob {
    const void* a[PS_MAX_PAIRS];
    const E2* b[PS_MAX_PAIRS];
    E2* fin_a[PS_MAX_PAIRS];
    E2* fin_b[PS_MAX_PAIRS];
    E2* bufa[2];
    E2* bufb[2];
    int npairs, nvars;
    int tail_rd;
    int tail_buf;
    size_t r_off;
    size_t sums_slot;
    int eq_n, eq_single;
    const E2* eq_scal;
    const E2* eq_lo;
    const E2* eq_suf;
    E2* bufA[2];
    E2* eqA0;
};
struct PsEqPoint {
    size_t point_off;
    int w, nvars;
    unsigned hib;
    int kmin;
    E2* lo;
    E2* suf;
};
inline int ps_eq_kmin(int nvars) { int k = nvars - 13 < 9 ? nvars - 13 : 9; return k < 0 ? 0 : k; }
inline size_t ps_eq_lo_entries(int nvars) { return nvars > 8 ? (size_t)(nvars - 8) * 384 : 0; }
inline size_t ps_eq_suf_entries(int nvars) { return ((size_t)2 << (nvars - ps_eq_kmin(nvars))) - 1; }
constexpr int PS_EQ_MAX_VARS = 26;
void ps_eq_prep(hipStream_t st, const PsEqPoint* pts, int npts, const E2* chal);
void ps_eq_A(hipStream_t st, const PsJob* jobs, const int* ids, int nids, size_t max_quads);
struct PsItem {
    int job, jb_log2, blk0, nblk;
    int rd;
    int in_buf, out_buf;
    int pad;
};
int ps_plan_blocks(PsItem* items, int nitems, const PsJob* host_jobs, bool rounds2);
void ps_round(hipStream_t st, bool rounds2, const PsJob* jobs, const PsItem* items, int nitems, int grid, const E2* chal, E2* partials, E2* res, bool eq = false);
void ps_tail(hipStream_t st, const PsJob* jobs, int njobs, const E2* chal, E2* res);
size_t ps_tail_items_max();

struct ScatterEnt { const E2* src; size_t dst; };
void scatter_e2(hipStream_t st, const ScatterEnt* ents, size_t n, E2* dst_base);
void set_e2(hipStream_t st, E2* dst, E2 v);
void stamp(hipStream_t st, unsigned long long* slot);
struct ClearSet { unsigned* p[4]; size_t n[4]; };
void clear_words(hipStream_t st, const ClearSet& c);

void reduce_partials(hipStream_t st, const E2* partials, int nblocks, int nv, E2* out);

struct EqJob {
    E2* out;
    int n;
    const E2* point_dev;
    ClaimSet cs;
    E2* ab;
    int blk0, rows;
    int pblk0;
};
void eq_jobs(hipStream_t st, const EqJob* jobs, int njobs, int max_n, const E2* chal);
__host__ __device__ inline size_t eq_ab_entries(int n) { return 256 + ((size_t)1 << (n > 8 ? n - 8 : 0)); }
struct EqAbGrid { int prep, fill; };
EqAbGrid eq_ab_plan(EqJob* host_jobs, int njobs);
void eq_jobs_ab(hipStream_t st, const EqJob* jobs, int njobs, EqAbGrid grid, const E2* chal);
void eq_jobs_prep(hipStream_t st, const EqJob* jobs, int njobs, EqAbGrid grid, const E2* chal);
void sum_tables(hipStream_t st, E2* out, const E2* tabs, int ntabs, size_t n);

struct LassoDev {
    int nu, alpha, num_lookups, seg_shift;
    size_t rows;
    const uint8_t* seg_lookup;
    u64 lookup_mask[32];
    u64 lookup_uses[32];
    int mem_dim[32];
    u32 mem_cutoff[32];
    u64 mpow[5];
    int lookup_nmems[32];
    int lookup_mems[32][4];
    int cnt_nsegs[4];
    uint8_t cnt_segs[4][128];
};
struct LimbSrc { const u64* input; const uint8_t* seg_lookup; int seg_shift; size_t rows; u64 lookup_mask[32]; };
LimbSrc limb_src(const LassoDev& L, const u64* input);
inline bool limbs_from_input_ok(const LassoDev& L) { return L.seg_shift >= 1 && (L.rows & (((size_t)1 << L.seg_shift) - 1)) == 0; }
struct EpRows { signed char row[32]; };
EpRows ep_rows_all(int alpha);
void lasso_dims(hipStream_t st, const LassoDev& L, const u64* input, u64* dims);
struct ColPow { u64 v[32]; };
void lasso_split(hipStream_t st, const LassoDev& L, const u64* input, u64* dims, u64* e_polys, const EpRows& rows, const ColPow* colpow = nullptr,
                 u64* col = nullptr);
size_t lasso_counter_temp_bytes(size_t n);
void lasso_counters(hipStream_t st, const LassoDev& L, int m, const u64* dims, u64* read_ts, u64* final_cts,
                    void* temp, size_t temp_bytes, u32* keys, u32* keys_sorted, u32* rows_in, u32* rows_sorted, u32* starts);
struct CounterOut { u64* read_ts[4]; u64* final_cts[4]; };
size_t lasso_counters_all_elems(const LassoDev& L, unsigned chunk_mask);
size_t lasso_counters_all_temp_bytes(size_t n_elems);
void lasso_counters_all(hipStream_t st, const LassoDev& L, unsigned chunk_mask, const u64* dims, const CounterOut& out, void* temp, size_t temp_bytes,
                        u32* keys, u32* keys_sorted, u32* vals, u32* vals_sorted, u32* starts , const u64* input = nullptr);
int lasso_claim(hipStream_t st, const LassoDev& L, const E2* eq, const u64* e_polys, const EpRows& rows, E2* partials);
int lasso_claim_in(hipStream_t st, const LassoDev& L, const E2* eq, const u64* input, u32 own, E2* partials, bool eq_is_ab = false);
constexpr int HASH_RW_MAX = 8;
struct HashRwArgs { const u64* ep[HASH_RW_MAX]; u64* rd[HASH_RW_MAX]; u64* wr[HASH_RW_MAX]; u64* rd1[HASH_RW_MAX]; u64* wr1[HASH_RW_MAX]; };
void lasso_hash_rw(hipStream_t st, size_t n, const u64* dim, const u64* read_ts, const HashRwArgs& args, int nmem, u64 gamma, u64 tau,
                   const LimbSrc* limbs = nullptr, int chunk = 0);
struct HashIfArgs { u32 cutoff[32]; const u64* fc[32]; int row_init[32], row_fin[32]; };
void lasso_hash_if(hipStream_t st, const HashIfArgs& args, int G, u64 gamma, u64 tau, u64* H2);
void prod_level(hipStream_t st, const u64* in, size_t in_len, u64* out, int nb);
void prod_level3(hipStream_t st, const u64* in, size_t in_len, u64* o1, u64* o2, u64* o3, int nb);
constexpr int PROD_TAIL_LEN = 2048;
struct ProdTailOut { u64* p[12]; };
void prod_tail(hipStream_t st, const u64* in, int in_len, const ProdTailOut& outs, int nlevels, int nb);
void gp_top(hipStream_t st, const u64* top, int nb, E2* roots, E2* evals);
void dot_eq(hipStream_t st, const E2* eq, const u64* const tabs[8], int ntab, size_t n, E2* partials, E2* out);
constexpr int DOT_MAX = 64;
struct DotTabs { const u64* t[DOT_MAX]; int slot[DOT_MAX]; signed char emem[DOT_MAX]; };
struct DotVirt {
    const u64* input; const uint8_t* seg_lookup; int seg_shift; size_t rows;
    u64 lookup_mask[32]; u64 lookup_uses[32]; int mem_dim[32]; u32 mem_cutoff[32];
};
void dot_eq_many(hipStream_t st, const E2* eq, const DotTabs& tabs, int ntab, size_t n, E2* partials, E2* out, const DotVirt* virt = nullptr);
bool open_x_takes_ab(const DotTabs& tabs, int ntab, size_t n, const DotVirt& virt);
bool open_x(hipStream_t st, const E2* eq, const DotTabs& tabs, int ntab, size_t n, E2* partials, E2* out, const DotVirt& virt, bool eq_is_ab = false);
void dot_eq_ab(hipStream_t st, const E2* ab, int nvars, const u64* tab, E2* partials, E2* out);

struct CsrLin { const u32* ptr; const u32* gate; const u64* coef; };
struct CsrMul { const u32* ptr; const u32* gate; const u64* coef; const u32* other_in; const u32* other_j; };
struct GatherT {
    CsrLin lin; CsrMul mul;
    const u64* in_vals[PS_MAX_PAIRS];
};
struct GatherJob { GatherT g; const E2* eqc; int log2_S, log2_G, log2_R; E2* T; };
void gather_jobs(hipStream_t st, const GatherJob* jobs, int njobs, size_t max_total);
struct GatherSeg { u32 lo, hi; int goff; int other_in; int joff; int pad; u64 coef; };
struct GatherSegJob { const GatherSeg* segs; int nseg; const E2* eqc; int log2_S, log2_G, log2_R; E2* T; const u64* in_vals[PS_MAX_PAIRS]; int blk0; };
void gather_seg_jobs(hipStream_t st, const GatherSegJob* jobs, int njobs, int grid);
int gather_seg_plan(GatherSegJob* host_jobs, int njobs);
void vanilla_gather_B(hipStream_t st, const CsrMul& mulR, const E2* eqc, const E2* eqx, const E2* u, int log2_S, int log2_G, int log2_R, E2* B);
struct GatherBJob { CsrMul m; const E2* eqc; const E2* eqx; const E2* u; int log2_S, log2_G, log2_R; E2* B; };
void gather_B_jobs(hipStream_t st, const GatherBJob* jobs, int njobs, size_t max_total);
int vanilla_const_sum(hipStream_t st, const u32* gate, const u64* coef, size_t nterms, const E2* eqc, int log2_G, int log2_R, E2* partials);
struct FftJob { E2* out; const u64* W; u64 scale; int L; ClaimSet cs; };
void fft_jobs(hipStream_t st, const FftJob* jobs, int njobs, int max_L, int max_claims, const E2* chal, E2* tab);
int fft_jobs_launches(int max_L);
void powers_table(hipStream_t st, u64* W, u64 w, size_t n);

struct EvalNode {
    const u32* lptr; const u32* lin_in; const u32* lin_j; const u64* lcoef;
    const u32* mptr; const u32* mi0; const u32* mj0; const u32* mi1; const u32* mj1; const u64* mcoef;
    const u64* w0;
    const u64* in[PS_MAX_PAIRS];
    u64* out;
    int log2_G, log2_S, log2_R;
    u32 num_gates;
};
void gate_eval(hipStream_t st, const EvalNode& n);

void ntt_batch(hipStream_t st, u64* data, int log2n, size_t batch, const u64* W, u64 scale, u64* scratch);
inline bool ntt_four_step(int log2n, const u64* scratch) { return log2n >= 8 && log2n <= 16 && scratch != nullptr; }
inline int ntt_radix2_grid(int log2n, size_t batch) { return (int)std::min<size_t>(((batch << (log2n - 1)) + 255) / 256, 4096); }

constexpr int DRV_MAX_K = 16;
constexpr u32 DRV_NONCANONICAL = 1, DRV_BOUND = 2, DRV_PADDING = 4, DRV_INEXACT = 8;
constexpr int DRV_FLAG_WORDS = 6 * DRV_MAX_K;
struct DeriveMod { u64 q, d, v, qinv, half, k0, r1_bound, r2_bound; int sh; int pad; };
struct DeriveArgs {
    const u64* s; const u64* e; const u64* k1;
    const u64* ais[DRV_MAX_K];
    u64* r1is[DRV_MAX_K];
    u64* r2is;
    u64* ct0is;
    u64* X;
    u32* flags;
    DeriveMod mod[DRV_MAX_K];
    u64 s_bound, e_bound, k1_bound;
    int n_log2, k;
};
void derive_unpack(hipStream_t st, const DeriveArgs& a);
void derive_pack(hipStream_t st, const DeriveArgs& a, const int64_t* compact);
void derive_mul(hipStream_t st, u64* X, int log2_len, int batch);
void derive_combine(hipStream_t st, const DeriveArgs& a);

}
}
```

hyper-greco_amd/csrc/prover_sumcheck.inc:

```

    static constexpr size_t TAIL_ITEMS = 4096;

    bool hash_recomp = false;
    std::vector<dev::StJob> st_jobs;
    std::vector<int> st_seq;
    std::vector<SlotPlan> st_slot;
    std::vector<int> st_credit_ntab;
    std::vector<double> st_fused_bytes;
    std::vector<std::function<void()>> st_after_seq;
    double pending_level_design = 0, pending_hash_reads = -1, hash_design_reads = 0;
    std::vector<double> st_level_design, st_hash_reads;
    double pending_fused_bytes = 0;
    double pending_fused_model_extra = 0, hash_model_extra = 0;
    std::vector<double> st_fused_model_extra;
    std::vector<dev::ScatterEnt> scatter;
    struct GpEpReq { int job = -1; dev::GpClaimEp ep; std::vector<E2> winv, gnext; };
    std::vector<GpEpReq> gp_eps;

    ScHandle sc_stride(int kind, const void* in, bool base, size_t in_stride, int ntab, int nvars, const dev::Powers& pw, E2* final_out,
                       bool enqueue = true, bool p0_only = false, int seq = 0, u64* next_level = nullptr, const dev::GpHashSrc* hash_src = nullptr,
                       const MirrorSpec* mirror = nullptr, int model_ntab = 0, const SlotPlan* slots = nullptr) {
        ScHandle h;
        h.nv = kind == dev::SC_GRANDPROD ? 3 : 2;
        h.nvars = nvars;
        h.point_off = epos();
        h.sums_slot = slot((size_t)nvars * h.nv);
        const size_t N = (size_t)1 << nvars;
        if (!enqueue) {
            pending_fused_bytes = 0; pending_fused_model_extra = 0; pending_level_design = 0; pending_hash_reads = -1;
            for (int i = 0; i < nvars; i++) h.rs.push_back(squeeze());
            return h;
        }
        dev::StJob J;
        memset(&J, 0, sizeof(J));
        J.in = in; J.in_stride = in_stride;
        J.buf[0] = ctx->alloc_n<E2>((size_t)ntab * std::max<size_t>(N / 2, 1));
        J.buf[1] = ctx->alloc_n<E2>((size_t)ntab * std::max<size_t>(N / 4, 1));
        J.final_out = final_out ? final_out : ctx->alloc_n<E2>(ntab);
        J.kind = kind; J.ntab = ntab; J.nvars = nvars; J.base = base ? 1 : 0; J.p0_only = p0_only ? 1 : 0;
        J.r_off = h.point_off; J.sums_slot = h.sums_slot;
        J.next_level = next_level; J.hash_src = hash_src;
        if (mirror) { J.mirror = 1; J.mk1 = mirror->k1; J.mk2 = mirror->k2; }
        if (slots && slots->job_slotw) { J.slotw = slots->job_slotw; J.emit_mask = slots->job_emit; J.slot_ng = slots->npairs; J.slot_shift = slots->max_rd; }
        memcpy(J.pw, pw.v, sizeof(J.pw));
        for (int i = 0; i < nvars; i++) h.rs.push_back(squeeze());
        if (nvars > 0)
            for (int i = 0; i < dev::PW_MAX; i++) J.pwr[i] = e2_mul(pw.v[i], h.rs[0]);
        if (nvars > 0) {
            st_slot.push_back(slots ? *slots : SlotPlan());
            st_jobs.push_back(J); st_seq.push_back(seq); st_credit_ntab.push_back(mirror ? mirror->credit_ntab : (model_ntab ? model_ntab : ntab));
            double fused = next_level ? (double)(st_credit_ntab.back() / 2) * (double)(2 * N) * 8.0 * (hash_src ? 0.5 : 1.5) : 0.0;
            st_fused_bytes.push_back(fused + pending_fused_bytes);
            st_fused_model_extra.push_back(pending_fused_model_extra);
            st_level_design.push_back(next_level ? pending_level_design : 0.0);
            st_hash_reads.push_back(hash_src ? pending_hash_reads : -1.0);
            pending_fused_bytes = 0; pending_fused_model_extra = 0; pending_level_design = 0; pending_hash_reads = -1;
        }
        return h;
    }

    static int slot_tail_h(int tail_ntab, int nvars) { return std::min(dev::st_tail_h(tail_ntab, nvars), nvars - 2); }
    void flush_stride() {
        if (st_jobs.empty()) return;
        const int nj = (int)st_jobs.size();
        if (hoist_consts)
            for (auto& J : st_jobs) {
                const size_t N = (size_t)1 << J.nvars;
                kept_writes(crange(J.buf[0], (size_t)J.ntab * std::max<size_t>(N / 2, 1)));
                kept_writes(crange(J.buf[1], (size_t)J.ntab * std::max<size_t>(N / 4, 1)));
                kept_writes(crange(J.final_out, (size_t)J.ntab));
            }
        constexpr int fuse_min_h = 15;
        struct Launch { int kind; bool base; int h_log2; bool tail; int nrounds; std::vector<dev::StItem> items; bool hash = false; bool after_seq = false;
                        int mode = 0;
        };
        std::vector<Launch> plan;
        struct Regroup { int job; const E2* in; E2* out; int len_log2; };
        std::vector<Regroup> regroups;
        std::vector<const void*> cur_in(nj);
        std::vector<size_t> cur_stride(nj);
        std::vector<int> next_h(nj);
        for (int q = 0; q < nj; q++) { cur_in[q] = st_jobs[q].in; cur_stride[q] = st_jobs[q].in_stride; next_h[q] = st_jobs[q].nvars - 1; }
        auto next_out = [&](int q) { return cur_in[q] == (const void*)st_jobs[q].buf[0] ? st_jobs[q].buf[1] : st_jobs[q].buf[0]; };
        std::vector<int> h_small(nj);
        for (int q = 0; q < nj; q++) {
            const SlotPlan& sp = st_slot[q];
            h_small[q] = sp.tail_ntab ? slot_tail_h(sp.tail_ntab, st_jobs[q].nvars) : dev::st_tail_h(st_jobs[q].ntab, st_jobs[q].nvars);
            if (st_seq[q] > 0) h_small[q] = std::min(h_small[q], st_jobs[q].nvars - 2);
            if (sp.tail_ntab && st_jobs[q].nvars - 1 - h_small[q] > sp.max_rd) throw Error("slot-form job: the tail starts below the segment pairs");
        }
        for (int kind : {dev::SC_COLLATION, dev::SC_GRANDPROD}) {
            int max_h = -1;
            for (auto& J : st_jobs) if (J.kind == kind) max_h = std::max(max_h, J.nvars - 1);
            if (max_h < 0) continue;
            if (kind == dev::SC_GRANDPROD) {
                int max_seq = 0;
                for (int q = 0; q < nj; q++) max_seq = std::max(max_seq, st_seq[q]);
                for (int sq = 1; sq <= max_seq; sq++)
                    for (int q = 0; q < nj; q++) {
                        const dev::StJob& J = st_jobs[q];
                        if (st_seq[q] != sq || J.kind != kind) continue;
                        if (!J.base || next_h[q] <= h_small[q]) throw Error("sequenced first round on a job that has none");
                        Launch ls{kind, true, -1, false, 1, {}};
                        ls.hash = J.hash_src != nullptr;
                        dev::StItem it;
                        memset(&it, 0, sizeof(it));
                        it.job = q; it.h_log2 = next_h[q]; it.in = cur_in[q]; it.in_stride = cur_stride[q]; it.out = J.buf[0];
                        ls.items.push_back(it);
                        cur_in[q] = it.out; cur_stride[q] = (size_t)1 << next_h[q];
                        next_h[q]--;
                        plan.push_back(ls);
                    }
                if (max_seq > 0 || !st_after_seq.empty()) { Launch la{kind, true, -1, false, 0, {}}; la.after_seq = true; plan.push_back(la); }
            }
            {
                Launch lall{kind, true, -1, false, 1, {}};
                for (int q = 0; q < nj; q++) {
                    const dev::StJob& J = st_jobs[q];
                    if (J.kind != kind || !J.base || next_h[q] <= h_small[q] || next_h[q] != J.nvars - 1) continue;
                    dev::StItem it;
                    memset(&it, 0, sizeof(it));
                    it.job = q; it.h_log2 = next_h[q]; it.in = cur_in[q]; it.in_stride = cur_stride[q]; it.out = J.buf[0];
                    lall.items.push_back(it);
                    cur_in[q] = it.out; cur_stride[q] = (size_t)1 << next_h[q];
                    next_h[q]--;
                }
                if (!lall.items.empty()) plan.push_back(lall);
            }
            static const bool no_split = hg_env_on("HG_NO_SPLIT");
            constexpr int split_h = 14;
            const bool may_split = kind == dev::SC_GRANDPROD && !no_split && st == ctx->stream && fork_recorded && world == 1;
            Launch lsum{kind, false, -1, false, 1, {}};
            lsum.mode = 2;
            for (;;) {
                Launch le{kind, false, -1, false, 1, {}}, l2{kind, false, -1, false, 2, {}};
                bool le_small = may_split;
                for (int q = 0; q < nj; q++) {
                    const dev::StJob& J = st_jobs[q];
                    const int h = next_h[q];
                    if (J.kind != kind || h <= h_small[q]) continue;
                    const bool first = J.nvars - 1 == h;
                    if (first && J.hash_src) throw Error("hash-source job without a sequenced first round");
                    dev::StItem it;
                    memset(&it, 0, sizeof(it));
                    it.job = q; it.h_log2 = h; it.in = cur_in[q]; it.in_stride = cur_stride[q];
                    it.out = first ? J.buf[0] : next_out(q);
                    const bool pair = !first && h - 1 > h_small[q] && h >= std::max(dev::ST_STEP2_MIN_H, fuse_min_h);
                    (pair ? l2 : le).items.push_back(it);
                    if (!pair && (first || h > split_h)) le_small = false;
                    next_h[q] = h - (pair ? 2 : 1);
                    cur_in[q] = it.out; cur_stride[q] = (size_t)1 << (pair ? h - 1 : h);
                }
                if (le.items.empty() && l2.items.empty()) break;
                if (!l2.items.empty()) plan.push_back(l2);
                if (!le.items.empty()) {
                    if (le_small) {
                        le.mode = 1;
                        for (auto& it : le.items) {
                            E2* fresh = ctx->alloc_n<E2>((size_t)st_jobs[it.job].ntab << it.h_log2);
                            it.out = fresh;
                            cur_in[it.job] = fresh;
                            lsum.items.push_back(it);
                        }
                    }
                    plan.push_back(le);
                }
            }
            if (!lsum.items.empty()) plan.push_back(lsum);
            {
                Launch lc{kind, false, 0, true, 0, {}};
                for (int q = 0; q < nj; q++) {
                    const dev::StJob& J = st_jobs[q];
                    if (J.kind != kind || next_h[q] < 0) continue;
                    const int hs = next_h[q];
                    dev::StItem it;
                    memset(&it, 0, sizeof(it));
                    it.job = q; it.in = cur_in[q]; it.in_stride = cur_stride[q];
                    it.rd = J.nvars - 1 - hs; it.nrounds = hs + 1; it.out = J.final_out;
                    if (st_slot[q].tail_ntab) {
                        const SlotPlan& sp = st_slot[q];
                        if (cur_stride[q] != (size_t)2 << hs) throw Error("slot-form job: unexpected table length at the tail");
                        E2* rg = ctx->alloc_n<E2>((size_t)sp.tail_ntab << (hs + 1));
                        regroups.push_back(Regroup{q, (const E2*)cur_in[q], rg, hs + 1});
                        it.in = rg; it.ntab = sp.tail_ntab;
                    }
                    lc.items.push_back(it);
                    next_h[q] = -1;
                }
                if (!lc.items.empty()) plan.push_back(lc);
            }
        }
        if (hg_debug("plan"))
            for (const Launch& L : plan) {
                if (L.after_seq) { fprintf(stderr, "[hg plan] stride kind=%d after_seq=1\n", L.kind); continue; }
                int lo = INT_MAX, hi = INT_MIN;
                for (const dev::StItem& it : L.items) { const int v = L.tail ? it.nrounds : it.h_log2; lo = std::min(lo, v); hi = std::max(hi, v); }
                fprintf(stderr, "[hg plan] stride kind=%d base=%d nrounds=%d mode=%d tail=%d hash=%d items=%zu %s=%d..%d\n", L.kind, L.base ? 1 : 0, L.nrounds,
                        L.mode, L.tail ? 1 : 0, L.hash ? 1 : 0, L.items.size(), L.tail ? "rounds" : "h", lo, hi);
            }
        if (!gp_eps.empty()) {
            std::vector<E2> wts;
            std::vector<dev::GpClaimEp> eps;
            for (const GpEpReq& e : gp_eps) {
                if (e.job < 0 || e.job >= nj || st_jobs[e.job].kind != dev::SC_GRANDPROD) throw Error("grand product: claim epilogue without its job");
                wts.insert(wts.end(), e.winv.begin(), e.winv.end());
                wts.insert(wts.end(), e.gnext.begin(), e.gnext.end());
            }
            E2* d_wts = ctx->alloc_n<E2>(wts.size());
            dev::GpClaimEp* d_eps = ctx->alloc_n<dev::GpClaimEp>(gp_eps.size());
            size_t o = 0;
            for (size_t i = 0; i < gp_eps.size(); i++) {
                dev::GpClaimEp ep = gp_eps[i].ep;
                ep.winv = d_wts + o; o += gp_eps[i].winv.size();
                ep.gnext = d_wts + o; o += gp_eps[i].gnext.size();
                eps.push_back(ep);
                st_jobs[gp_eps[i].job].ep = d_eps + i;
            }
            upload(d_wts, wts.data(), wts.size() * sizeof(E2), "upload claim weights");
            upload(d_eps, eps.data(), eps.size() * sizeof(dev::GpClaimEp), "upload claim epilogues");
            gp_eps.clear();
        }
        dev::StJob* d_jobs = ctx->alloc_n<dev::StJob>(nj);
        upload(d_jobs, st_jobs.data(), (size_t)nj * sizeof(dev::StJob), "upload jobs");
        std::vector<dev::StItem> flat;
        std::vector<size_t> offs;
        std::vector<std::vector<int>> grids(plan.size());
        for (size_t li = 0; li < plan.size(); li++) {
            Launch& L = plan[li];
            if (!L.tail && !L.after_seq)
                for (size_t o = 0; o < L.items.size(); o += MAX_BATCH)
                    grids[li].push_back(dev::st_plan_blocks(L.items.data() + o, (int)std::min<size_t>(MAX_BATCH, L.items.size() - o), L.nrounds == 2));
            offs.push_back(flat.size());
            flat.insert(flat.end(), L.items.begin(), L.items.end());
        }
        dev::StItem* d_items = ctx->alloc_n<dev::StItem>(flat.size());
        upload(d_items, flat.data(), flat.size() * sizeof(dev::StItem), "upload step items");
        auto round_bytes = [&](int q, int rd, bool model) {
            const dev::StJob& J = st_jobs[q];
            size_t half = (size_t)1 << (J.nvars - 1 - rd);
            return (double)(model ? st_credit_ntab[q] : J.ntab) * (2.0 * half * ((J.base && rd == 0) ? 8 : 16) + half * 16.0);
        };
        auto design_bytes = [&](int q, int rd, int nrounds, bool tail) {
            const dev::StJob& J = st_jobs[q];
            const size_t half = (size_t)1 << (J.nvars - 1 - rd);
            double b = (double)J.ntab * 2.0 * half * ((J.base && rd == 0) ? 8 : 16);
            if (rd == 0 && st_hash_reads[q] >= 0) b = st_hash_reads[q];
            if (!tail) b += (double)J.ntab * (double)(half >> (nrounds - 1)) * 16.0;
            if (rd == 0) b += st_level_design[q];
            return b;
        };
        for (size_t li = 0; li < plan.size(); li++) {
            const Launch& L = plan[li];
            if (L.kind == dev::SC_GRANDPROD && st_before_gp) { stamp("collation done"); st_before_gp(); st_before_gp = nullptr; stamp("grand products may start"); }
            if (L.after_seq) {
                for (auto& f : st_after_seq) f();
                st_after_seq.clear();
                if (st_before_gp2) { st_before_gp2(); st_before_gp2 = nullptr; }
                continue;
            }
            for (size_t o = 0; o < L.items.size(); o += MAX_BATCH) {
                const int cnt = (int)std::min<size_t>(MAX_BATCH, L.items.size() - o);
                double bytes = 0, model = 0;
                if (L.hash) {
                    const dev::StItem& it = L.items[o];
                    bytes = round_bytes(it.job, 0, false) + st_fused_bytes[it.job];
                    model = round_bytes(it.job, 0, true) + st_fused_bytes[it.job] + st_fused_model_extra[it.job];
                    ctx->prof_begin(cls_gp_hash, bytes, model, design_bytes(it.job, 0, 1, false));
                    dev::st_first_hash(st, d_jobs + it.job, d_items + offs[li] + o, grids[li][0], st_jobs[it.job].mirror != 0, hash_recomp, ctx->d_chal, partials, d_res(), st_slot[it.job].tail_ntab != 0);
                    ctx->prof_end();
                    stamp("first hash round done");
                    continue;
                }
                if (L.tail) {
                    size_t table_bytes = 0;
                    double design = 0;
                    std::vector<dev::SlotRegroupJob> rg_jobs;
                    size_t rg_max = 0;
                    for (int q = 0; q < cnt; q++) {
                        const dev::StItem& it = L.items[o + q];
                        const dev::StJob& J = st_jobs[it.job];
                        for (int k = 0; k < it.nrounds; k++) { bytes += round_bytes(it.job, it.rd + k, false); model += round_bytes(it.job, it.rd + k, true); }
                        design += (double)(it.ntab > 0 ? it.ntab : J.ntab) * 2.0 * (double)((size_t)1 << (J.nvars - 1 - it.rd)) * ((J.base && it.rd == 0) ? 8 : 16);
                        const int h0 = J.nvars - 1 - it.rd;
                        table_bytes = std::max(table_bytes, (size_t)(it.ntab > 0 ? it.ntab : J.ntab) * (((size_t)1 << h0) + (((size_t)1 << h0) >> 1)) * sizeof(E2));
                        for (const Regroup& g : regroups) if (g.job == it.job) {
                            const SlotPlan& sp = st_slot[it.job];
                            rg_jobs.push_back(dev::gp_slot_regroup_job(g.in, g.out, sp.d_slot_of, sp.d_ratio, sp.nrows, sp.nslots, sp.npairs, g.len_log2, (sp.tail_ntab & 1) != 0));
                            rg_max = std::max(rg_max, ((size_t)sp.nrows + (sp.tail_ntab & 1)) << g.len_log2);
                        }
                    }
                    if (!rg_jobs.empty()) {
                        dev::SlotRegroupJob* d_rg = ctx->alloc_n<dev::SlotRegroupJob>(rg_jobs.size());
                        upload(d_rg, rg_jobs.data(), rg_jobs.size() * sizeof(dev::SlotRegroupJob), "upload regroup jobs");
                        dev::gp_slot_regroup_jobs(st, d_rg, (int)rg_jobs.size(), rg_max);
                    }
                    ctx->prof_begin(cls_tail, bytes, model, design);
                    dev::st_tail(st, L.kind, d_jobs, d_items + offs[li] + o, cnt, table_bytes, ctx->d_chal, d_res());
                    ctx->prof_end();
                } else {
                    double design = 0;
                    for (int q = 0; q < cnt; q++) {
                        const dev::StItem& it = L.items[o + q];
                        const dev::StJob& J = st_jobs[it.job];
                        design += design_bytes(it.job, J.nvars - 1 - it.h_log2, L.nrounds, false);
                        for (int k = 0; k < L.nrounds; k++) { bytes += round_bytes(it.job, J.nvars - 1 - it.h_log2 + k, false); model += round_bytes(it.job, J.nvars - 1 - it.h_log2 + k, true); }
                        if (L.base && it.h_log2 == J.nvars - 1) { bytes += st_fused_bytes[it.job]; model += st_fused_bytes[it.job]; }
                    }
                    const int grid = grids[li][o / MAX_BATCH];
                    int cls = L.kind == dev::SC_GRANDPROD ? (L.base ? cls_gp_base : (L.nrounds == 2 ? cls_gp_ext2 : cls_gp_ext)) : (L.base ? cls_col_base : (L.nrounds == 2 ? cls_col_ext2 : cls_col_ext));
                    if (L.mode == 2) {
                        if (o == 0) {
                            hip_check(hipEventRecord(ctx->ev_sum[0], st), "split rounds: folds done");
                            hip_check(hipStreamWaitEvent(ctx->stream_sum, ctx->ev_sum[0], 0), "split rounds: wait for the folds");
                        }
                        ctx->prof_stream = ctx->stream_sum;
                        ctx->prof_begin(cls_gp_sums, 0, 0, design);
                        dev::st_step(ctx->stream_sum, L.kind, false, d_jobs, d_items + offs[li] + o, cnt, grid, ctx->d_chal, ctx->d_partials4, d_res(), false, 2);
                        ctx->prof_end();
                        ctx->prof_stream = st;
                        if (o + MAX_BATCH >= L.items.size()) {
                            hip_check(hipEventRecord(ctx->ev_sum[1], ctx->stream_sum), "split rounds: sums done");
                            ctx->sum_pending = true;
                        }
                        continue;
                    }
                    ctx->prof_begin(cls, bytes, model, design);
                    if (L.nrounds == 2) dev::st_step2(st, L.kind, d_jobs, d_items + offs[li] + o, cnt, grid, ctx->d_chal, partials, d_res());
                    else dev::st_step(st, L.kind, L.base, d_jobs, d_items + offs[li] + o, cnt, grid, ctx->d_chal, partials, d_res(),
                                      L.base && st_jobs[L.items[o].job].slotw != nullptr, L.mode);
                    ctx->prof_end();
                }
            }
        }
        if (st_before_gp) { st_before_gp(); st_before_gp = nullptr; }
        if (st_before_gp2) { st_before_gp2(); st_before_gp2 = nullptr; }
        st_jobs.clear();
        st_seq.clear();
        st_credit_ntab.clear();
        st_slot.clear();
        st_fused_bytes.clear();
        st_fused_model_extra.clear();
        st_level_design.clear();
        st_hash_reads.clear();
        for (auto& f : st_after_seq) f();
        st_after_seq.clear();
        if (!scatter.empty()) {
            dev::ScatterEnt* d = ctx->alloc_n<dev::ScatterEnt>(scatter.size());
            upload(d, scatter.data(), scatter.size() * sizeof(dev::ScatterEnt), "upload scatter list");
            dev::scatter_e2(st, d, scatter.size(), d_res());
            scatter.clear();
        }
    }

    std::map<int, std::vector<dev::PsJob>> ps_queue;
    std::vector<std::function<void()>> second_wave;

    ScHandle sc_prodsum(const std::vector<const u64*>& a, const std::vector<const E2*>& b, int nvars,
                        const std::vector<E2*>& fin_a, const std::vector<E2*>& fin_b, bool enqueue = true) {
        ScHandle h;
        h.nv = 2;
        h.nvars = nvars;
        h.point_off = epos();
        h.sums_slot = slot((size_t)nvars * 2);
        if (!enqueue) {
            for (int i = 0; i < nvars; i++) h.rs.push_back(squeeze());
            return h;
        }
        const int np = (int)a.size();
        if (np > dev::PS_MAX_PAIRS) throw Error("prodsum: too many table pairs");
        const size_t N = (size_t)1 << nvars;
        dev::PsJob J;
        memset(&J, 0, sizeof(J));
        J.npairs = np; J.nvars = nvars; J.r_off = h.point_off; J.sums_slot = h.sums_slot;
        for (int q = 0; q < 2; q++) {
            J.bufa[q] = ctx->alloc_n<E2>((size_t)np * std::max<size_t>(N >> (q + 1), 1));
            J.bufb[q] = ctx->alloc_n<E2>((size_t)np * std::max<size_t>(N >> (q + 1), 1));
        }
        for (int i = 0; i < np; i++) { J.a[i] = a[i]; J.b[i] = b[i]; J.fin_a[i] = fin_a[i]; J.fin_b[i] = fin_b[i]; }
        for (int i = 0; i < nvars; i++) h.rs.push_back(squeeze());
        ps_queue[nvars].push_back(J);
        return h;
    }
    static bool ps_eq_on() { static const bool v = !hg_env_on("HG_NO_PS_EQ"); return v; }
    static size_t ps_tail_items() { return std::min<size_t>(TAIL_ITEMS, dev::ps_tail_items_max()); }
    static int eq_tail_rd(int npairs, int nvars) {
        if (npairs < 1 || npairs > dev::PS_MAX_PAIRS || nvars > dev::PS_EQ_MAX_VARS) return -1;
        const size_t N = (size_t)1 << nvars;
        int rd = 0;
        while (rd < nvars && ((N >> rd) / 2) * (size_t)npairs > ps_tail_items()) rd++;
        if (rd & 1) rd++;
        if (rd < 2 || rd > nvars - 8 || rd < dev::ps_eq_kmin(nvars)) return -1;
        return rd;
    }
    std::vector<E2> eq_scal_host;
    std::vector<dev::PsEqPoint> eqpt_queue;
    std::map<std::tuple<size_t, int, int, unsigned>, std::pair<E2*, E2*>> eqpt_shared;
    ScHandle sc_prodsum_eq(const std::vector<const u64*>& a, const std::vector<E2>& kappa, const std::vector<E2>& zp, size_t z_off, int w, unsigned hib,
                           int nvars, int tail_rd, const std::vector<E2*>& fin_a, const std::vector<E2*>& fin_b, bool enqueue) {
        ScHandle h;
        h.nv = 2;
        h.nvars = nvars;
        h.point_off = epos();
        h.sums_slot = slot((size_t)nvars * 2);
        for (int i = 0; i < nvars; i++) h.rs.push_back(squeeze());
        if (!enqueue) return h;
        const int np = (int)a.size();
        const size_t N = (size_t)1 << nvars;
        dev::PsJob J;
        memset(&J, 0, sizeof(J));
        J.npairs = np; J.nvars = nvars; J.r_off = h.point_off; J.sums_slot = h.sums_slot;
        J.tail_rd = tail_rd; J.eq_n = np; J.eq_single = np == 1 ? 1 : 0;
        for (int q = 0; q < 2; q++) {
            J.bufa[q] = ctx->alloc_n<E2>((size_t)np * (N >> (q + 1)));
            if (np > 1) J.bufA[q] = ctx->alloc_n<E2>(N >> (q + 1));
        }
        if (np > 1) J.eqA0 = ctx->alloc_n<E2>(N);
        for (int i = 0; i < np; i++) { J.a[i] = a[i]; J.fin_a[i] = fin_a[i]; J.fin_b[i] = fin_b[i]; }
        std::vector<E2> scal((size_t)2 * nvars + 1 + np + nvars + 4 * (size_t)(tail_rd / 2), e2_zero());
        E2 P = e2_one();
        for (int rd = 0; rd <= tail_rd && rd < nvars; rd++) {
            if (rd == tail_rd) { scal[(size_t)2 * nvars] = P; break; }
            const E2 z = zp[rd], omz = e2_sub(e2_one(), z);
            E2 p0 = e2_mul(P, omz), p2 = e2_mul(P, e2_sub(e2_add(e2_dbl(z), z), e2_one()));
            if (np == 1) { p0 = e2_mul(p0, kappa[0]); p2 = e2_mul(p2, kappa[0]); }
            scal[(size_t)2 * rd] = p0; scal[(size_t)2 * rd + 1] = p2;
            P = e2_mul(P, e2_add(e2_mul(z, h.rs[rd]), e2_mul(omz, e2_sub(e2_one(), h.rs[rd]))));
        }
        for (int i = 0; i < np; i++) scal[(size_t)2 * nvars + 1 + i] = kappa[i];
        for (int k = 0; k < nvars; k++) scal[(size_t)2 * nvars + 1 + np + k] = zp[k];
        for (int rd = 0; rd + 1 < tail_rd; rd += 2) {
            const E2 ra = h.rs[rd], rb = h.rs[rd + 1], na = e2_sub(e2_one(), ra), nb = e2_sub(e2_one(), rb);
            E2* c = &scal[(size_t)2 * nvars + 1 + np + nvars + 4 * (size_t)(rd / 2)];
            c[0] = e2_mul(na, nb); c[1] = e2_mul(ra, nb); c[2] = e2_mul(na, rb); c[3] = e2_mul(ra, rb);
        }
        J.eq_scal = reinterpret_cast<const E2*>(eq_scal_host.size() * sizeof(E2));
        eq_scal_host.insert(eq_scal_host.end(), scal.begin(), scal.end());
        const auto key = std::make_tuple(z_off, w, nvars, hib);
        auto hit = eqpt_shared.find(key);
        if (hit == eqpt_shared.end()) {
            dev::PsEqPoint pt;
            memset(&pt, 0, sizeof(pt));
            pt.point_off = z_off; pt.w = w; pt.nvars = nvars; pt.hib = hib; pt.kmin = dev::ps_eq_kmin(nvars);
            pt.lo = ctx->alloc_n<E2>(dev::ps_eq_lo_entries(nvars));
            pt.suf = ctx->alloc_n<E2>(dev::ps_eq_suf_entries(nvars));
            eqpt_queue.push_back(pt);
            hit = eqpt_shared.emplace(key, std::make_pair(pt.lo, pt.suf)).first;
        }
        J.eq_lo = hit->second.first; J.eq_suf = hit->second.second;
        ps_queue[nvars].push_back(J);
        return h;
    }
    void flush_prodsum() {
        std::vector<dev::PsJob> jobs;
        for (auto& kv : ps_queue) { jobs.insert(jobs.end(), kv.second.begin(), kv.second.end()); kv.second.clear(); }
        if (jobs.empty()) return;
        const int nj = (int)jobs.size();
        if (hoist_consts)
            for (auto& J : jobs) {
                const size_t N = (size_t)1 << J.nvars;
                for (int q = 0; q < 2; q++) {
                    const size_t len = std::max<size_t>(N >> (q + 1), 1);
                    kept_writes(crange(J.bufa[q], (size_t)J.npairs * len));
                    kept_writes(crange(J.bufb[q], (size_t)J.npairs * len));
                    kept_writes(crange(J.bufA[q], len));
                }
                kept_writes(crange(J.eqA0, N));
            }
        if (hg_debug("eq")) {
            int ne = 0; size_t ee = 0, et = 0;
            for (auto& J : jobs) { const size_t e = (size_t)J.npairs << J.nvars; et += e; if (J.eq_n) { ne++; ee += e; } }
            fprintf(stderr, "[hg eq] %d of %d queued node reductions eq-factored, %zu of %zu table entries\n", ne, nj, ee, et);
        }
        if (!eq_scal_host.empty()) {
            E2* d_scal = ctx->alloc_n<E2>(eq_scal_host.size());
            upload(d_scal, eq_scal_host.data(), eq_scal_host.size() * sizeof(E2), "upload eq-form scalars");
            for (auto& J : jobs) if (J.eq_n) J.eq_scal = d_scal + reinterpret_cast<size_t>(J.eq_scal) / sizeof(E2);
            eq_scal_host.clear();
        }
        int max_rd = 0;
        for (auto& J : jobs) {
            const size_t N = (size_t)1 << J.nvars;
            int rd = 0;
            if (J.eq_n) rd = J.tail_rd;
            else while (rd < J.nvars && ((N >> rd) / 2) * (size_t)J.npairs > ps_tail_items()) rd++;
            J.tail_rd = rd;
            max_rd = std::max(max_rd, rd);
        }
        auto round_bytes = [&](const dev::PsJob& J, int rd) {
            size_t half = ((size_t)1 << J.nvars) >> (rd + 1);
            if (J.eq_n && rd < J.tail_rd)
                return (double)J.npairs * (2.0 * half * (rd == 0 ? 8 : 16) + half * 16.0) + (J.eq_single ? 0.0 : (rd == 0 ? 0.0 : 2.0 * half * 16) + half * 16.0);
            return (double)J.npairs * (2.0 * half * ((rd == 0 ? 8 : 16) + 16) + half * 32.0);
        };
        constexpr int ps_fuse_min_h = 9;
        auto design_bytes = [&](const dev::PsJob& J, int rd, int nrounds) {
            const size_t half = ((size_t)1 << J.nvars) >> (rd + 1), out = half >> (nrounds - 1);
            const double ea = rd == 0 ? 8 : 16;
            if (J.eq_n) return (double)J.npairs * (2.0 * half * ea + out * 16.0) + (J.eq_single ? 0.0 : 2.0 * half * 16.0 + out * 16.0);
            return (double)J.npairs * (2.0 * half * (ea + 16) + out * 32.0);
        };
        struct PsLaunch { bool two, eq; int cnt, grid; size_t off; double bytes, design; };
        std::vector<PsLaunch> launches;
        std::vector<dev::PsItem> all_items;
        std::vector<int> next_rd(nj, 0), cur_buf(nj, -1);
        for (;;) {
            std::vector<dev::PsItem> one, two, two_eq;
            for (int q = 0; q < nj; q++) {
                const dev::PsJob& J = jobs[q];
                const int rd = next_rd[q];
                if (rd >= J.tail_rd) continue;
                const int h = J.nvars - 1 - rd;
                const bool pair = J.eq_n ? true : rd + 1 < J.tail_rd && h >= std::max(9, ps_fuse_min_h);
                dev::PsItem it;
                memset(&it, 0, sizeof(it));
                it.job = q; it.rd = rd; it.in_buf = cur_buf[q]; it.out_buf = cur_buf[q] == 1 ? 0 : 1;
                if (cur_buf[q] < 0) it.out_buf = pair ? 1 : 0;
                if (J.eq_n && rd + 2 >= J.tail_rd) it.pad = 1;
                (J.eq_n ? two_eq : pair ? two : one).push_back(it);
                next_rd[q] = rd + (pair ? 2 : 1);
                cur_buf[q] = it.out_buf;
            }
            if (one.empty() && two.empty() && two_eq.empty()) break;
            for (int kind = 0; kind < 3; kind++) {
                std::vector<dev::PsItem>& items = kind == 0 ? two_eq : kind == 1 ? one : two;
                const bool fused = kind != 1;
                for (size_t o = 0; o < items.size(); o += MAX_BATCH) {
                    const int cnt = (int)std::min<size_t>(MAX_BATCH, items.size() - o);
                    const int grid = dev::ps_plan_blocks(items.data() + o, cnt, jobs.data(), fused);
                    double bytes = 0, design = 0;
                    for (int q = 0; q < cnt; q++) {
                        for (int k = 0; k <= (fused ? 1 : 0); k++) bytes += round_bytes(jobs[items[o + q].job], items[o + q].rd + k);
                        design += design_bytes(jobs[items[o + q].job], items[o + q].rd, fused ? 2 : 1);
                    }
                    launches.push_back({fused, kind == 0, cnt, grid, all_items.size(), bytes, design});
                    all_items.insert(all_items.end(), items.begin() + o, items.begin() + o + cnt);
                }
            }
        }
        for (int q = 0; q < nj; q++) jobs[q].tail_buf = cur_buf[q];
        if (hg_debug("plan")) {
            for (const PsLaunch& L : launches) {
                int lo = INT_MAX, hi = INT_MIN;
                std::string hs;
                for (int q = 0; q < L.cnt; q++) {
                    const dev::PsItem& it = all_items[L.off + q];
                    lo = std::min(lo, it.rd); hi = std::max(hi, it.rd);
                    hs += (q ? "," : "") + std::to_string(jobs[it.job].nvars - 1 - it.rd);
                }
                fprintf(stderr, "[hg plan] prodsum two=%d eq=%d cnt=%d rd=%d..%d h=[%s]\n", L.two ? 1 : 0, L.eq ? 1 : 0, L.cnt, lo, hi, hs.c_str());
            }
            int lo = INT_MAX, hi = INT_MIN;
            for (auto& J : jobs) { lo = std::min(lo, J.tail_rd); hi = std::max(hi, J.tail_rd); }
            fprintf(stderr, "[hg plan] prodsum tail jobs=%d tail_rd=%d..%d\n", nj, lo, hi);
        }
        dev::PsJob* d_jobs = ctx->alloc_n<dev::PsJob>(nj);
        upload(d_jobs, jobs.data(), (size_t)nj * sizeof(dev::PsJob), "upload jobs");
        {
            std::vector<int> ids;
            size_t max_quads = 0; double ab = 0;
            for (int q = 0; q < nj; q++) if (jobs[q].eq_n > 1) {
                ids.push_back(q);
                const size_t N = (size_t)1 << jobs[q].nvars;
                max_quads = std::max(max_quads, N >> 2);
                ab += (double)N * (8.0 * jobs[q].eq_n + 16.0);
            }
            if (!ids.empty()) {
                int* d_ids = ctx->alloc_n<int>(ids.size());
                upload(d_ids, ids.data(), ids.size() * sizeof(int), "upload eq-form job list");
                ctx->prof_begin(cls_aux, ab);
                dev::ps_eq_A(st, d_jobs, d_ids, (int)ids.size(), max_quads);
                ctx->prof_end();
            }
        }
        if (!all_items.empty()) {
            dev::PsItem* d_items = ctx->alloc_n<dev::PsItem>(all_items.size());
            upload(d_items, all_items.data(), all_items.size() * sizeof(dev::PsItem), "upload items");
            for (auto& L : launches) {
                ctx->prof_begin(L.two ? cls_ps2 : cls_ps, L.bytes, -1.0, L.design);
                dev::ps_round(st, L.two, d_jobs, d_items + L.off, L.cnt, L.grid, ctx->d_chal, partials, d_res(), L.eq);
                ctx->prof_end();
            }
        }
        double tb = 0, td = 0;
        for (auto& J : jobs) {
            for (int rd = J.tail_rd; rd < J.nvars; rd++) tb += round_bytes(J, rd);
            if (J.tail_rd < J.nvars) {
                const size_t half = ((size_t)1 << J.nvars) >> (J.tail_rd + 1);
                td += (double)J.npairs * 2.0 * half * (J.tail_rd == 0 ? 8 : 16) + (J.eq_n ? 2.0 * half * 16 : (double)J.npairs * 2.0 * half * 16);
            }
        }
        ctx->prof_begin(cls_ps_tail, tb, -1.0, td);
        dev::ps_tail(st, d_jobs, nj, ctx->d_chal, d_res());
        ctx->prof_end();
    }
    static constexpr size_t MAX_BATCH = 64;
    bool defer_uploads = false;
    struct Upload { void* dst; const void* src; size_t bytes; };
    std::vector<Upload> deferred_uploads;
    void upload(void* dst, const void* src, size_t bytes, const char* what) {
        const void* staged = stage(src, bytes);
        if (defer_uploads) { deferred_uploads.push_back(Upload{dst, staged, bytes}); return; }
        hip_check(hipMemcpyAsync(dst, staged, bytes, hipMemcpyHostToDevice, st), what);
    }
    bool hoist_consts = false;
    struct ConstRange { const char* lo; const char* hi; };
    std::vector<std::function<void(hipStream_t)>> hoisted;
    std::vector<ConstRange> hoisted_ranges, kept_ranges;
    std::vector<const void*> key_allocs;
    int n_hoisted = 0, n_split = 0;
    size_t hoisted_bytes = 0;
    template <typename T> static ConstRange crange(const T* p, size_t n) {
        return ConstRange{reinterpret_cast<const char*>(p), reinterpret_cast<const char*>(p) + n * sizeof(T)};
    }
    bool in_hoisted(ConstRange r) const {
        for (const ConstRange& h : hoisted_ranges) if (r.lo < h.hi && h.lo < r.hi) return true;
        return false;
    }
    bool const_src(const void* p) const {
        if (!p) return true;
        if (std::binary_search(key_allocs.begin(), key_allocs.end(), p, std::less<const void*>())) return true;
        const char* c = static_cast<const char*>(p);
        return in_hoisted(ConstRange{c, c + 1});
    }
    void kept_writes(ConstRange r) const {
        if (hoist_consts && r.lo && r.lo < r.hi && in_hoisted(r)) throw Error("launch graph: a recorded launch writes a table that was built once");
    }
    template <typename Fn> void issue_const(bool constant, const std::vector<ConstRange>& writes, int nlaunch, Fn fn) {
        if (!(hoist_consts && constant)) {
            for (const ConstRange& w : writes) { kept_writes(w); if (hoist_consts && w.lo && w.lo < w.hi) kept_ranges.push_back(w); }
            fn(st);
            return;
        }
        for (const ConstRange& w : writes) {
            if (!w.lo || w.lo >= w.hi) continue;
            bool clash = in_hoisted(w);
            for (const ConstRange& k : kept_ranges) clash = clash || (w.lo < k.hi && k.lo < w.hi);
// ... 236 lines not shown
```

Baseline: 1.487 ms.

## Fold-first tail rounds and paired split-sum launches for grand-product endgame

The grand-product tail kernel gains a fold-first mode. It runs only one or two whole rounds, then performs all remaining folds into LDS level buffers before computing every round's sums in a single pass with combined cross-wave reductions, which removes per-round sync and reduction overhead. The split-sums stream now pairs consecutive rounds of the same job into one k_st_step2<SUMS> launch that skips the fold stores, with a wider item lookup of up to 128 items, which cuts launch count. This adds considerable complexity and different LDS sizing. An env flag can restore the old tail path.

```diff
diff --git a/hyper-greco_amd/csrc/kernels.hip b/hyper-greco_amd/csrc/kernels.hip
--- a/hyper-greco_amd/csrc/kernels.hip
+++ b/hyper-greco_amd/csrc/kernels.hip
@@ -241,7 +241,7 @@
     const u64 z = 0, u = __builtin_nondeterministic_value(z);
     return GpItemE2{e2(u, u), e2(u, u), e2(u, u), e2(u, u)};
 }
-template <int KIND, typename T, bool FIRST, bool SLOT = false, bool GIO = true, int MODE = 0>
+template <int KIND, typename T, bool FIRST, bool SLOT = false, bool GIO = true, int MODE = 0, bool GOUT = GIO>
 __device__ __forceinline__ void sc_round_body(const T* __restrict__ in, size_t in_stride, E2* __restrict__ out,
                                               size_t out_stride, int ntab, size_t half, E2 r, const E2* __restrict__ pw, const E2* __restrict__ pwr,
                                               int jb_log2, E2* __restrict__ red, E2* acc, size_t first_tile, size_t tile_step,
@@ -289,8 +289,8 @@
                         we2_mac(wi, dl, dr);
                     }
                     if (MODE != 2) {
-                        store_e2<GIO>(out + (size_t)(2 * i) * out_stride + jo, e2_fold_wide(xl, dl, fr));
-                        store_e2<GIO>(out + (size_t)(2 * i + 1) * out_stride + jo, e2_fold_wide(xr, dr, fr));
+                        store_e2<GOUT>(out + (size_t)(2 * i) * out_stride + jo, e2_fold_wide(xl, dl, fr));
+                        store_e2<GOUT>(out + (size_t)(2 * i + 1) * out_stride + jo, e2_fold_wide(xr, dr, fr));
                     }
                     gp_cur = nxt;
                 }
@@ -302,7 +302,7 @@
                         s0 = e2_add(s0, e2_add(e2_mul(mirror->mk1, x), mirror->mk2));
                         s2 = e2_add(s2, e2_add(e2_mul(mirror->mk1, y), mirror->mk2));
                     }
-                    if (MODE != 2) store_e2<GIO>(out + (size_t)(2 * nb) * out_stride + jo, e2_fold_wide(x, e2_sub(y, x), fr));
+                    if (MODE != 2) store_e2<GOUT>(out + (size_t)(2 * nb) * out_stride + jo, e2_fold_wide(x, e2_sub(y, x), fr));
                 }
             } else {
             for (int i = g; i < nb; i += G) {
@@ -520,6 +520,12 @@
     const unsigned long long m = __ballot(b0 <= blk);
     return __builtin_amdgcn_readfirstlane(__popcll(m) - 1);
 }
+__device__ __forceinline__ int find_item128(const StItem* __restrict__ items, int nitems, int blk) {
+    const int l = threadIdx.x & 63;
+    const int b0 = l < nitems ? items[l].blk0 : 0x7fffffff, b1 = l + 64 < nitems ? items[l + 64].blk0 : 0x7fffffff;
+    const unsigned long long m0 = __ballot(b0 <= blk), m1 = __ballot(b1 <= blk);
+    return __builtin_amdgcn_readfirstlane(__popcll(m0) + __popcll(m1) - 1);
+}
 template <int KIND, typename T, bool SLOT = false, int MODE = 0>
 __global__ __launch_bounds__(256) void k_st_step(const StJob* __restrict__ jobs, const StItem* __restrict__ items, int nitems,
                                                  const E2* __restrict__ chal, E2* __restrict__ partials, E2* __restrict__ res) {
@@ -920,12 +926,37 @@
     a2 = e2_add(a2, e2_mul(q3, p3));
     return q2;
 }
+template <bool SUMS = false>
 __global__ __launch_bounds__(256) void k_st_step2(const StJob* __restrict__ jobs, const StItem* __restrict__ items, int nitems,
                                                   const E2* __restrict__ chal, E2* __restrict__ partials, E2* __restrict__ res) {
-    const int y = find_item(items, nitems, blockIdx.x);
+    const int y = SUMS ? find_item128(items, nitems, blockIdx.x) : find_item(items, nitems, blockIdx.x);
     const StItem& I = items[y];
     const StJob& J = jobs[I.job];
     const int h_log2 = I.h_log2;
+    constexpr size_t PSTRIDE = SUMS ? (size_t)ST_SUMS_PART_BLOCKS * 6 : (size_t)SC_MAX_BLOCKS * 6;
+    constexpr int TSTRIDE = SUMS ? 16 : 32;
+    if constexpr (SUMS) {
+        if (I.nrounds != 2) {
+            const int rd1 = J.nvars - 1 - h_log2;
+            const size_t half1 = (size_t)1 << h_log2;
+            const int nblk1 = I.nblk, bx1 = (int)blockIdx.x - I.blk0;
+            E2* sm1 = dyn_lds;
+            E2 acc1[3] = {e2_zero(), e2_zero(), e2_zero()};
+            sc_round_body<SC_GRANDPROD, E2, false, false, true, 2>(reinterpret_cast<const E2*>(I.in), I.in_stride, I.out, half1, J.ntab, half1, chal[J.r_off + rd1], J.pw, J.pwr, I.jb_log2,
+                                                                   dyn_lds + SM_SLOTS, acc1, bx1, nblk1, J.p0_only != 0, nullptr, J.mirror ? &J : nullptr);
+            E2* part1 = partials + (size_t)y * PSTRIDE;
+            block_sum_multi<3>(acc1, sm1);
+            if (threadIdx.x == 0) {
+#pragma unroll
+                for (int t = 0; t < 3; t++) {
+                    if (nblk1 == 1) res[J.sums_slot + (size_t)rd1 * 3 + t] = acc1[t];
+                    else part_store(part1 + (size_t)bx1 * 3 + t, acc1[t]);
+                }
+            }
+            if (nblk1 > 1) finish_partials(part1, 3, tickets_of(partials) + y * TSTRIDE, res + J.sums_slot + (size_t)rd1 * 3, sm1, nblk1);
+            return;
+        }
+    }
     const int rd = J.nvars - 1 - h_log2;
     const size_t half = (size_t)1 << h_log2, half2 = half >> 1;
     const size_t ntiles = half >> 8;
@@ -965,8 +996,10 @@
             w0.A.L = c0.c0; w0.C.L = c0.c1;
             w1.A.L = c1.c0; w1.C.L = c1.c1;
             vm.c0.L = cm.c0; vm.c1.L = cm.c1;
-            const E2 fs = e2_fold_wide(ms, es, fb);
-            if (!odd) store_e2(out + (size_t)(2 * nb) * half2 + jo2, fs);
+            if constexpr (!SUMS) {
+                const E2 fs = e2_fold_wide(ms, es, fb);
+                if (!odd) store_e2(out + (size_t)(2 * nb) * half2 + jo2, fs);
+            }
         }
         for (int i = 0; i < nb; i++) {
             const bool more_i = i + 1 < nb, more_t = tile + nblocks < ntiles;
@@ -996,8 +1029,10 @@
                 const u64 c = odd ? el.c1 : gl_mul7_lazy(el.c1);
                 wmac_pair(vi, el.c0, b, c, d);
             }
-            const E2 fx = odd ? mr : ml, fd = odd ? er : el;
-            store_e2(out + (size_t)(2 * i + (odd ? 1 : 0)) * half2 + jo2, e2_fold_wide(fx, fd, fb));
+            if constexpr (!SUMS) {
+                const E2 fx = odd ? mr : ml, fd = odd ? er : el;
+                store_e2(out + (size_t)(2 * i + (odd ? 1 : 0)) * half2 + jo2, e2_fold_wide(fx, fd, fb));
+            }
             cur = nxt;
         }
         gp_combine(we2_reduce(w0), we2_reduce(w1), we2_reduce(wi), p0, p2, p3, acc[0], acc[1], acc[2]);
@@ -1006,7 +1041,7 @@
         if (!odd) gp_combine(mine, other, e2(ip, iq), q0, q2, q3, acc[3], acc[4], acc[5]);
     }
     E2* sm = dyn_lds;
-    E2* part = partials + (size_t)y * SC_MAX_BLOCKS * 6;
+    E2* part = partials + (size_t)y * PSTRIDE;
     block_sum_multi<6>(acc, sm);
     if (threadIdx.x == 0) {
 #pragma unroll
@@ -1015,7 +1050,7 @@
             else part_store(part + (size_t)bx * 6 + t, acc[t]);
         }
     }
-    if (nblocks > 1) finish_partials(part, 6, tickets_of(partials) + y * 32, res + J.sums_slot + (size_t)rd * 3, sm, nblocks);
+    if (nblocks > 1) finish_partials(part, 6, tickets_of(partials) + y * TSTRIDE, res + J.sums_slot + (size_t)rd * 3, sm, nblocks);
 }
 __global__ __launch_bounds__(256) void k_col_step2(const StJob* __restrict__ jobs, const StItem* __restrict__ items, int nitems,
                                                    const E2* __restrict__ chal, E2* __restrict__ partials, E2* __restrict__ res) {
@@ -1117,7 +1152,7 @@
         if (threadIdx.x == 0) gstore_e2(res + ep->next_slot, s);
     }
 }
-template <int KIND>
+template <int KIND, bool FF = false>
 __global__ __launch_bounds__(ST_TAIL_THREADS) void k_st_tail(const StJob* __restrict__ jobs, const StItem* __restrict__ items, const E2* __restrict__ chal,
                                                  E2* __restrict__ res) {
     constexpr int NV = KIND == SC_GRANDPROD ? 3 : 2;
@@ -1148,8 +1183,12 @@
     __shared__ E2 keep[3 * 32], rch[32];
     if ((int)threadIdx.x < J.nvars - I.rd) rch[threadIdx.x] = chal[J.r_off + I.rd + threadIdx.x];
     __syncthreads();
+    const int R = J.nvars - I.rd;
+    int whole = R;
+    if constexpr (FF) whole = ((size_t)(2 * J.ntab) << h0) * sizeof(E2) <= ST_TAIL_LDS_BYTES ? 1 : 2;
+    if (whole > R) whole = R;
 #pragma unroll 1
-    for (int rd = I.rd; rd < J.nvars; rd++) {
+    for (int rd = I.rd; rd < I.rd + whole; rd++) {
         const int h_log2 = J.nvars - 1 - rd;
         const size_t half = (size_t)1 << h_log2;
         const int jb_log2 = h_log2 < 8 ? h_log2 : 8;
@@ -1160,7 +1199,10 @@
         const E2 r = rch[rd - I.rd];
         if (rd == 0 && J.base) sc_round_body<KIND, u64, true, false, false>(reinterpret_cast<const u64*>(in), in_stride, out, half, J.ntab, half, r, J.pw, J.pwr, jb_log2, red, acc, 0, 1, p0_only);
         else if (rd == 0) sc_round_body<KIND, E2, true, false, false>(reinterpret_cast<const E2*>(in), in_stride, out, half, J.ntab, half, r, J.pw, J.pwr, jb_log2, red, acc, 0, 1, p0_only);
-        else sc_round_body<KIND, E2, false, false, false>(reinterpret_cast<const E2*>(in), in_stride, out, half, J.ntab, half, r, J.pw, J.pwr, jb_log2, red, acc, 0, 1, p0_only, nullptr, mirror);
+        else if constexpr (FF) {
+            if (rd == I.rd) sc_round_body<KIND, E2, false, false, true, 0, false>(reinterpret_cast<const E2*>(in), in_stride, out, half, J.ntab, half, r, J.pw, J.pwr, jb_log2, red, acc, 0, 1, p0_only, nullptr, mirror);
+            else sc_round_body<KIND, E2, false, false, false>(reinterpret_cast<const E2*>(in), in_stride, out, half, J.ntab, half, r, J.pw, J.pwr, jb_log2, red, acc, 0, 1, p0_only, nullptr, mirror);
+        } else sc_round_body<KIND, E2, false, false, false>(reinterpret_cast<const E2*>(in), in_stride, out, half, J.ntab, half, r, J.pw, J.pwr, jb_log2, red, acc, 0, 1, p0_only, nullptr, mirror);
         block_sum_multi<NV>(acc, sm);
         if (threadIdx.x == 0) {
 #pragma unroll
@@ -1168,6 +1210,122 @@
         }
         __syncthreads();
         in = out; in_stride = half;
+    }
+    if constexpr (FF && KIND == SC_GRANDPROD) if (whole < R) {
+        const int ntab = J.ntab, nb = ntab >> 1, tid = threadIdx.x, lane = tid & 63, wave = tid >> 6;
+        E2* const ffb = whole == 1 ? tab[1] : tab[0];
+        auto lvl = [&](int k) -> E2* {
+            return k < whole ? tab[k & 1] : ffb + (size_t)ntab * (((size_t)2 << (h0 - whole)) - ((size_t)2 << (h0 - k)));
+        };
+#pragma unroll 1
+        for (int k = whole; k < R; k++) {
+            const int hl = h0 - k;
+            const size_t half = (size_t)1 << hl;
+            const E2* __restrict__ src = lvl(k - 1);
+            E2* __restrict__ dst = lvl(k);
+            const FoldR fr = fold_r(rch[k]);
+            for (size_t e = tid; e < ((size_t)ntab << hl); e += ST_TAIL_THREADS) {
+                const size_t i = e >> hl, j = e & (half - 1);
+                const E2 x = src[i * 2 * half + j], y = src[i * 2 * half + half + j];
+                dst[i * half + dpos(j, half)] = e2_fold_wide(x, e2_sub(y, x), fr);
+            }
+            __syncthreads();
+        }
+        const bool mir = mirror != nullptr;
+        const E2 mk1 = J.mk1, mk2 = J.mk2;
+#pragma unroll 1
+        for (int k = whole; k < R; k++) {
+            const int hl = h0 - k;
+            const size_t half = (size_t)1 << hl, ts = 2 * half;
+            const E2* __restrict__ src = lvl(k - 1);
+            if (hl >= 6) {
+                E2 a[3] = {e2_zero(), e2_zero(), e2_zero()};
+                for (size_t j = tid; j < half; j += ST_TAIL_THREADS) {
+                    WE2 w0 = we2_zero(), w1 = we2_zero(), wi = we2_zero();
+                    E2 p0 = e2_zero(), p2 = e2_zero(), p3 = e2_zero();
+                    for (int i = 0; i < nb; i++) {
+                        const E2* tl = src + (size_t)(2 * i) * ts + j;
+                        const E2 xl = tl[0], yl = tl[half], xr = tl[ts], yr = tl[ts + half];
+                        const E2 dl = e2_sub(yl, xl), dr = e2_sub(yr, xr);
+                        if (i == 0) { p0 = xl; p2 = e2_add(yl, dl); p3 = e2_add(p2, dl); }
+                        if (!(p0_only && i == 0)) { we2_mac(w0, xl, xr); we2_mac(w1, yl, yr); we2_mac(wi, dl, dr); }
+                    }
+                    E2 s0 = we2_reduce(w0), s2 = we2_reduce(w1);
+                    if (mir) {
+                        const E2* tl = src + (size_t)(2 * nb) * ts + j;
+                        s0 = e2_add(s0, e2_add(e2_mul(mk1, tl[0]), mk2));
+                        s2 = e2_add(s2, e2_add(e2_mul(mk1, tl[half]), mk2));
+                    }
+                    gp_combine(s0, s2, we2_reduce(wi), p0, p2, p3, a[0], a[1], a[2]);
+                }
+#pragma unroll
+                for (int c = 0; c < 3; c++) {
+                    a[c] = wave_sum(a[c]);
+                    if (lane == 0) sm[((hl - 6) * 4 + wave) * 3 + c] = a[c];
+                }
+            } else {
+                const int JB = 1 << hl, jj = tid & (JB - 1), g = tid >> hl, G = ST_TAIL_THREADS >> hl;
+                WE2 w0 = we2_zero(), w1 = we2_zero(), wi = we2_zero();
+                for (int i = g; i < nb; i += G) {
+                    const E2* tl = src + (size_t)(2 * i) * ts + jj;
+                    const E2 xl = tl[0], yl = tl[half], xr = tl[ts], yr = tl[ts + half];
+                    if (!(p0_only && i == 0)) { we2_mac(w0, xl, xr); we2_mac(w1, yl, yr); we2_mac(wi, e2_sub(yl, xl), e2_sub(yr, xr)); }
+                }
+                E2 s[3] = {we2_reduce(w0), we2_reduce(w1), we2_reduce(wi)};
+                for (int m = 32; m >= JB; m >>= 1) {
+#pragma unroll
+                    for (int c = 0; c < 3; c++) s[c] = e2_add(s[c], e2(__shfl_xor((unsigned long long)s[c].c0, m, 64), __shfl_xor((unsigned long long)s[c].c1, m, 64)));
+                }
+                if ((lane >> hl) == 0) {
+#pragma unroll
+                    for (int c = 0; c < 3; c++) red[(4 * (JB - 1) + wave * JB + jj) * 3 + c] = s[c];
+                }
+            }
+        }
+        __syncthreads();
+        if (tid < 64) {
+            const int hl = tid ? 31 - __clz(tid) : 0;
+            const int JB = 1 << hl, jj = tid - JB, k = h0 - hl;
+            const bool on = tid > 0 && k >= whole;
+            E2 v[3] = {e2_zero(), e2_zero(), e2_zero()};
+            if (on) {
+                E2 s[3] = {e2_zero(), e2_zero(), e2_zero()};
+                for (int w = 0; w < ST_TAIL_THREADS / 64; w++) {
+#pragma unroll
+                    for (int c = 0; c < 3; c++) s[c] = e2_add(s[c], red[(4 * (JB - 1) + w * JB + jj) * 3 + c]);
+                }
+                const size_t half = (size_t)JB, ts = 2 * half;
+                const E2* __restrict__ src = lvl(k - 1);
+                const E2 xl = src[jj], yl = src[half + jj], dl = e2_sub(yl, xl);
+                const E2 p2 = e2_add(yl, dl);
+                if (mir) {
+                    const E2* tl = src + (size_t)(2 * nb) * ts + jj;
+                    s[0] = e2_add(s[0], e2_add(e2_mul(mk1, tl[0]), mk2));
+                    s[1] = e2_add(s[1], e2_add(e2_mul(mk1, tl[half]), mk2));
+                }
+                gp_combine(s[0], s[1], s[2], xl, p2, e2_add(p2, dl), v[0], v[1], v[2]);
+            }
+            for (int b = 0; b < 5; b++) {
+#pragma unroll
+                for (int c = 0; c < 3; c++) {
+                    const E2 o = e2(__shfl_xor((unsigned long long)v[c].c0, 1 << b, 64), __shfl_xor((unsigned long long)v[c].c1, 1 << b, 64));
+                    if (b < hl) v[c] = e2_add(v[c], o);
+                }
+            }
+            if (on && jj == 0) {
+#pragma unroll
+                for (int c = 0; c < 3; c++) keep[k * 3 + c] = v[c];
+            }
+        } else if (tid < 64 + 15) {
+            const int hb = (tid - 64) / 3, c = (tid - 64) % 3, k = h0 - (hb + 6);
+            if (k >= whole) {
+                E2 s = e2_zero();
+                for (int w = 0; w < ST_TAIL_THREADS / 64; w++) s = e2_add(s, sm[(hb * 4 + w) * 3 + c]);
+                keep[k * 3 + c] = s;
+            }
+        }
+        __syncthreads();
+        in = lvl(R - 1);
     }
     if ((int)threadIdx.x < (J.nvars - I.rd) * NV) res[J.sums_slot + (size_t)I.rd * NV + threadIdx.x] = keep[threadIdx.x];
     const E2* fin = reinterpret_cast<const E2*>(in);
@@ -1220,12 +1378,19 @@
     const size_t n = ((size_t)nrows + (has_s ? 1 : 0)) << len_log2;
     k_gp_slot_regroup<<<(unsigned)((n + 255) / 256), 256, 0, st>>>(in, out, slot_of, ratio, nrows, nslots, npairs, len_log2, len_log2 - np_log2, has_s ? 1 : 0);
 }
-void st_tail(hipStream_t st, int kind, const StJob* jobs, const StItem* items, int nitems, size_t table_bytes, const E2* chal, E2* res) {
+int st_tail_whole_rounds(int ntab, int h0) { return ((size_t)(2 * ntab) << h0) * sizeof(E2) <= ST_TAIL_LDS_BYTES ? 1 : 2; }
+size_t st_tail_table_bytes(int ntab, int h0, bool fold_first) {
+    const size_t l0 = (size_t)ntab << h0;
+    return (fold_first && h0 >= 1 && st_tail_whole_rounds(ntab, h0) == 1 ? 2 * l0 : l0 + (l0 >> 1)) * sizeof(E2);
+}
+void st_tail(hipStream_t st, int kind, const StJob* jobs, const StItem* items, int nitems, size_t table_bytes, const E2* chal, E2* res, bool fold_first) {
     const size_t lds = (SM_SLOTS + 3 * ST_TAIL_THREADS) * sizeof(E2) + table_bytes;
     static const hipError_t a1 = hipFuncSetAttribute((const void*)k_st_tail<SC_GRANDPROD>, hipFuncAttributeMaxDynamicSharedMemorySize, (int)((SM_SLOTS + 3 * ST_TAIL_THREADS) * sizeof(E2) + ST_TAIL_LDS_BYTES));
     static const hipError_t a2 = hipFuncSetAttribute((const void*)k_st_tail<SC_COLLATION>, hipFuncAttributeMaxDynamicSharedMemorySize, (int)((SM_SLOTS + 3 * ST_TAIL_THREADS) * sizeof(E2) + ST_TAIL_LDS_BYTES));
-    (void)a1; (void)a2;
-    if (kind == SC_GRANDPROD) k_st_tail<SC_GRANDPROD><<<nitems, ST_TAIL_THREADS, lds, st>>>(jobs, items, chal, res);
+    static const hipError_t a3 = hipFuncSetAttribute((const void*)k_st_tail<SC_GRANDPROD, true>, hipFuncAttributeMaxDynamicSharedMemorySize, (int)((SM_SLOTS + 3 * ST_TAIL_THREADS) * sizeof(E2) + ST_TAIL_LDS_BYTES));
+    (void)a1; (void)a2; (void)a3;
+    if (kind == SC_GRANDPROD && fold_first) k_st_tail<SC_GRANDPROD, true><<<nitems, ST_TAIL_THREADS, lds, st>>>(jobs, items, chal, res);
+    else if (kind == SC_GRANDPROD) k_st_tail<SC_GRANDPROD><<<nitems, ST_TAIL_THREADS, lds, st>>>(jobs, items, chal, res);
     else k_st_tail<SC_COLLATION><<<nitems, ST_TAIL_THREADS, lds, st>>>(jobs, items, chal, res);
 }
 
@@ -1236,7 +1401,7 @@
     for (int q = 0; q < nitems; q++) {
         StItem& I = items[q];
         int jb = 8;
-        if (!rounds2) while (jb > 2 && (total << (8 - jb)) < st_min_threads()) jb--;
+        if (!rounds2 && I.nrounds != 2) while (jb > 2 && (total << (8 - jb)) < st_min_threads()) jb--;
         if (jb > I.h_log2) jb = I.h_log2;
         const size_t ntiles = ((size_t)1 << I.h_log2) >> jb;
         I.jb_log2 = jb;
@@ -1268,8 +1433,14 @@
     }
 }
 void st_step2(hipStream_t st, int kind, const StJob* jobs, const StItem* items, int nitems, int grid, const E2* chal, E2* partials, E2* res) {
-    if (kind == SC_GRANDPROD) k_st_step2<<<grid, 256, sc_lds_bytes(0, 256), st>>>(jobs, items, nitems, chal, partials, res);
+    if (kind == SC_GRANDPROD) k_st_step2<false><<<grid, 256, sc_lds_bytes(0, 256), st>>>(jobs, items, nitems, chal, partials, res);
     else k_col_step2<<<grid, 256, sc_lds_bytes(0, 256), st>>>(jobs, items, nitems, chal, partials, res);
+}
+static_assert(HG_TEST_ST_MAX_BLOCKS <= ST_SUMS_PART_BLOCKS && (size_t)ST_SUMS_MAX_ITEMS * ST_SUMS_PART_BLOCKS * 6 <= PARTIALS_E2 && ST_SUMS_MAX_ITEMS * 16 <= PARTIALS_TICKETS,
+              "st_sums: the items of a launch share one partials buffer");
+void st_sums(hipStream_t st, const StJob* jobs, const StItem* items, int nitems, int grid, const E2* chal, E2* partials, E2* res) {
+    if (nitems > ST_SUMS_MAX_ITEMS) throw std::runtime_error("st_sums: too many items in one launch");
+    k_st_step2<true><<<grid, 256, sc_lds_bytes(3, 256), st>>>(jobs, items, nitems, chal, partials, res);
 }
 __device__ __forceinline__ void ps_io(const PsJob& J, int rd, int rounds, int in_buf, int out_buf, int i, const void*& a, const E2*& b, E2*& oa, E2*& ob) {
     const size_t N = (size_t)1 << J.nvars;
diff --git a/hyper-greco_amd/csrc/kernels.hpp b/hyper-greco_amd/csrc/kernels.hpp
--- a/hyper-greco_amd/csrc/kernels.hpp
+++ b/hyper-greco_amd/csrc/kernels.hpp
@@ -102,8 +102,13 @@
              E2* partials, E2* res, bool slot = false, int mode = 0);
 void st_first_hash(hipStream_t st, const StJob* job, const StItem* item, int grid, bool mirror, bool recomp, const E2* chal, E2* partials, E2* res, bool slot = false);
 void st_step2(hipStream_t st, int kind, const StJob* jobs, const StItem* items, int nitems, int grid, const E2* chal, E2* partials, E2* res);
+constexpr int ST_SUMS_MAX_ITEMS = 128, ST_SUMS_PART_BLOCKS = 512;
+void st_sums(hipStream_t st, const StJob* jobs, const StItem* items, int nitems, int grid, const E2* chal, E2* partials, E2* res);
 int st_tail_h(int ntab, int nvars);
-void st_tail(hipStream_t st, int kind, const StJob* jobs, const StItem* items, int nitems, size_t table_bytes, const E2* chal, E2* res);
+int st_tail_whole_rounds(int ntab, int h0);
+size_t st_tail_table_bytes(int ntab, int h0, bool fold_first);
+void st_tail(hipStream_t st, int kind, const StJob* jobs, const StItem* items, int nitems, size_t table_bytes, const E2* chal, E2* res, bool fold_first = false);
+constexpr int ST_SUMS_PAIR_MAX_NB = 24;
 constexpr int ST_STEP2_MIN_H = 9;
 
 struct PsJob {
diff --git a/hyper-greco_amd/csrc/prover_sumcheck.inc b/hyper-greco_amd/csrc/prover_sumcheck.inc
--- a/hyper-greco_amd/csrc/prover_sumcheck.inc
+++ b/hyper-greco_amd/csrc/prover_sumcheck.inc
@@ -73,7 +73,9 @@
         constexpr int fuse_min_h = 15;
         struct Launch { int kind; bool base; int h_log2; bool tail; int nrounds; std::vector<dev::StItem> items; bool hash = false; bool after_seq = false;
                         int mode = 0;
+                        std::vector<dev::StItem> run;
         };
+        int n_tail_ff = 0, n_tail_whole = 0, n_sum_pairs = 0, n_sum_singles = 0;
         std::vector<Launch> plan;
         struct Regroup { int job; const E2* in; E2* out; int len_log2; };
         std::vector<Regroup> regroups;
@@ -166,7 +168,20 @@
                     plan.push_back(le);
                 }
             }
-            if (!lsum.items.empty()) plan.push_back(lsum);
+            if (!lsum.items.empty()) {
+                if (!hg_env_on("HG_SUMS_SINGLE")) {
+                    std::vector<dev::StItem> byjob = lsum.items;
+                    std::stable_sort(byjob.begin(), byjob.end(), [](const dev::StItem& a, const dev::StItem& b) { return a.job < b.job; });
+                    for (size_t k = 0; k < byjob.size(); k++) {
+                        dev::StItem it = byjob[k];
+                        if (k + 1 < byjob.size() && byjob[k + 1].job == it.job && byjob[k + 1].h_log2 == it.h_log2 - 1 && it.h_log2 >= dev::ST_STEP2_MIN_H &&
+                            st_jobs[it.job].ntab / 2 <= dev::ST_SUMS_PAIR_MAX_NB) { it.nrounds = 2; k++; n_sum_pairs++; }
+                        else n_sum_singles++;
+                        lsum.run.push_back(it);
+                    }
+                } else n_sum_singles += (int)lsum.items.size();
+                plan.push_back(lsum);
+            }
             {
                 Launch lc{kind, false, 0, true, 0, {}};
                 for (int q = 0; q < nj; q++) {
@@ -227,11 +242,13 @@
         std::vector<std::vector<int>> grids(plan.size());
         for (size_t li = 0; li < plan.size(); li++) {
             Launch& L = plan[li];
+            std::vector<dev::StItem>& its = L.run.empty() ? L.items : L.run;
+            const size_t batch = L.run.empty() ? MAX_BATCH : (size_t)dev::ST_SUMS_MAX_ITEMS;
             if (!L.tail && !L.after_seq)
-                for (size_t o = 0; o < L.items.size(); o += MAX_BATCH)
-                    grids[li].push_back(dev::st_plan_blocks(L.items.data() + o, (int)std::min<size_t>(MAX_BATCH, L.items.size() - o), L.nrounds == 2));
+                for (size_t o = 0; o < its.size(); o += batch)
+                    grids[li].push_back(dev::st_plan_blocks(its.data() + o, (int)std::min<size_t>(batch, its.size() - o), L.nrounds == 2));
             offs.push_back(flat.size());
-            flat.insert(flat.end(), L.items.begin(), L.items.end());
+            flat.insert(flat.end(), its.begin(), its.end());
         }
         dev::StItem* d_items = ctx->alloc_n<dev::StItem>(flat.size());
         upload(d_items, flat.data(), flat.size() * sizeof(dev::StItem), "upload step items");
@@ -258,11 +275,13 @@
                 if (st_before_gp2) { st_before_gp2(); st_before_gp2 = nullptr; }
                 continue;
             }
-            for (size_t o = 0; o < L.items.size(); o += MAX_BATCH) {
-                const int cnt = (int)std::min<size_t>(MAX_BATCH, L.items.size() - o);
+            const std::vector<dev::StItem>& its = L.run.empty() ? L.items : L.run;
+            const size_t batch = L.run.empty() ? MAX_BATCH : (size_t)dev::ST_SUMS_MAX_ITEMS;
+            for (size_t o = 0; o < its.size(); o += batch) {
+                const int cnt = (int)std::min<size_t>(batch, its.size() - o);
                 double bytes = 0, model = 0;
                 if (L.hash) {
-                    const dev::StItem& it = L.items[o];
+                    const dev::StItem& it = its[o];
                     bytes = round_bytes(it.job, 0, false) + st_fused_bytes[it.job];
                     model = round_bytes(it.job, 0, true) + st_fused_bytes[it.job] + st_fused_model_extra[it.job];
                     ctx->prof_begin(cls_gp_hash, bytes, model, design_bytes(it.job, 0, 1, false));
@@ -274,15 +293,18 @@
                 if (L.tail) {
                     size_t table_bytes = 0;
                     double design = 0;
+                    const bool tail_ff = L.kind == dev::SC_GRANDPROD && !hg_env_on("HG_TAIL_WHOLE_ROUNDS");
                     std::vector<dev::SlotRegroupJob> rg_jobs;
                     size_t rg_max = 0;
                     for (int q = 0; q < cnt; q++) {
-                        const dev::StItem& it = L.items[o + q];
+                        const dev::StItem& it = its[o + q];
                         const dev::StJob& J = st_jobs[it.job];
                         for (int k = 0; k < it.nrounds; k++) { bytes += round_bytes(it.job, it.rd + k, false); model += round_bytes(it.job, it.rd + k, true); }
                         design += (double)(it.ntab > 0 ? it.ntab : J.ntab) * 2.0 * (double)((size_t)1 << (J.nvars - 1 - it.rd)) * ((J.base && it.rd == 0) ? 8 : 16);
-                        const int h0 = J.nvars - 1 - it.rd;
-                        table_bytes = std::max(table_bytes, (size_t)(it.ntab > 0 ? it.ntab : J.ntab) * (((size_t)1 << h0) + (((size_t)1 << h0) >> 1)) * sizeof(E2));
+                        const int h0 = J.nvars - 1 - it.rd, tn = it.ntab > 0 ? it.ntab : J.ntab;
+                        table_bytes = std::max(table_bytes, dev::st_tail_table_bytes(tn, h0, tail_ff));
+                        if (tail_ff && it.nrounds > dev::st_tail_whole_rounds(tn, h0)) n_tail_ff++;
+                        else if (L.kind == dev::SC_GRANDPROD) n_tail_whole++;
                         for (const Regroup& g : regroups) if (g.job == it.job) {
                             const SlotPlan& sp = st_slot[it.job];
                             rg_jobs.push_back(dev::gp_slot_regroup_job(g.in, g.out, sp.d_slot_of, sp.d_ratio, sp.nrows, sp.nslots, sp.npairs, g.len_log2, (sp.tail_ntab & 1) != 0));
@@ -295,18 +317,18 @@
                         dev::gp_slot_regroup_jobs(st, d_rg, (int)rg_jobs.size(), rg_max);
                     }
                     ctx->prof_begin(cls_tail, bytes, model, design);
-                    dev::st_tail(st, L.kind, d_jobs, d_items + offs[li] + o, cnt, table_bytes, ctx->d_chal, d_res());
+                    dev::st_tail(st, L.kind, d_jobs, d_items + offs[li] + o, cnt, table_bytes, ctx->d_chal, d_res(), tail_ff);
                     ctx->prof_end();
                 } else {
                     double design = 0;
                     for (int q = 0; q < cnt; q++) {
-                        const dev::StItem& it = L.items[o + q];
+                        const dev::StItem& it = its[o + q];
                         const dev::StJob& J = st_jobs[it.job];
                         design += design_bytes(it.job, J.nvars - 1 - it.h_log2, L.nrounds, false);
                         for (int k = 0; k < L.nrounds; k++) { bytes += round_bytes(it.job, J.nvars - 1 - it.h_log2 + k, false); model += round_bytes(it.job, J.nvars - 1 - it.h_log2 + k, true); }
                         if (L.base && it.h_log2 == J.nvars - 1) { bytes += st_fused_bytes[it.job]; model += st_fused_bytes[it.job]; }
                     }
-                    const int grid = grids[li][o / MAX_BATCH];
+                    const int grid = grids[li][o / batch];
                     int cls = L.kind == dev::SC_GRANDPROD ? (L.base ? cls_gp_base : (L.nrounds == 2 ? cls_gp_ext2 : cls_gp_ext)) : (L.base ? cls_col_base : (L.nrounds == 2 ? cls_col_ext2 : cls_col_ext));
                     if (L.mode == 2) {
                         if (o == 0) {
@@ -315,10 +337,11 @@
                         }
                         ctx->prof_stream = ctx->stream_sum;
                         ctx->prof_begin(cls_gp_sums, 0, 0, design);
-                        dev::st_step(ctx->stream_sum, L.kind, false, d_jobs, d_items + offs[li] + o, cnt, grid, ctx->d_chal, ctx->d_partials4, d_res(), false, 2);
+                        if (!L.run.empty()) dev::st_sums(ctx->stream_sum, d_jobs, d_items + offs[li] + o, cnt, grid, ctx->d_chal, ctx->d_partials4, d_res());
+                        else dev::st_step(ctx->stream_sum, L.kind, false, d_jobs, d_items + offs[li] + o, cnt, grid, ctx->d_chal, ctx->d_partials4, d_res(), false, 2);
                         ctx->prof_end();
                         ctx->prof_stream = st;
-                        if (o + MAX_BATCH >= L.items.size()) {
+                        if (o + batch >= its.size()) {
                             hip_check(hipEventRecord(ctx->ev_sum[1], ctx->stream_sum), "split rounds: sums done");
                             ctx->sum_pending = true;
                         }
@@ -327,11 +350,13 @@
                     ctx->prof_begin(cls, bytes, model, design);
                     if (L.nrounds == 2) dev::st_step2(st, L.kind, d_jobs, d_items + offs[li] + o, cnt, grid, ctx->d_chal, partials, d_res());
                     else dev::st_step(st, L.kind, L.base, d_jobs, d_items + offs[li] + o, cnt, grid, ctx->d_chal, partials, d_res(),
-                                      L.base && st_jobs[L.items[o].job].slotw != nullptr, L.mode);
+                                      L.base && st_jobs[its[o].job].slotw != nullptr, L.mode);
                     ctx->prof_end();
                 }
             }
         }
+        if (hg_debug("endgame") && (n_tail_ff || n_tail_whole || n_sum_pairs || n_sum_singles))
+            fprintf(stderr, "[hg endgame] stride tail_fold_first=%d tail_whole=%d sums_pairs=%d sums_singles=%d\n", n_tail_ff, n_tail_whole, n_sum_pairs, n_sum_singles);
         if (st_before_gp) { st_before_gp(); st_before_gp = nullptr; }
         if (st_before_gp2) { st_before_gp2(); st_before_gp2 = nullptr; }
         st_jobs.clear();
```

New measurement: 1.451 ms, median of 6. 2.5% less time.
